# ucla-mobility/QuantV2X

Hardware: AMD Instinct MI355X
Metric: frames/sec/node (N-agent int8 BEV fusion) (higher is better)
Workload: dtype i8

## Files before the change

### include/qv2x.h

```cpp
#ifndef QV2X_H
#define QV2X_H

#include <stdint.h>

#ifdef __cplusplus
extern "C" {
#endif
#if defined(__GNUC__) || defined(__clang__)
#pragma GCC visibility push(default)
#endif

#define QV2X_OK 0
#define QV2X_EINVAL (-1)
#define QV2X_EALIGN (-2)
#define QV2X_MAX_GROUPS 4

const char* qv2x_last_error(void);
#define QV2X_ABI_VERSION 9
int qv2x_version(void);

int qv2x_fill_i8(int8_t* buf, int64_t bytes, int value, void* stream);

int64_t qv2x_voxelize_workspace_bytes(int n_points);
int qv2x_voxelize_f32(const float* points, int n_points, const float* lidar_range, const float* voxel_size, int agent,
                      int max_points, int max_voxels, void* workspace, int64_t workspace_bytes,
                      float* voxel_features, int32_t* voxel_coords, int32_t* voxel_num_points, int32_t* n_voxels, void* stream);

int64_t qv2x_voxelize_batch_workspace_bytes(int n_sweeps, const int32_t* n_points );
int qv2x_voxelize_batch_f32(const float* const* points , const int32_t* n_points , int n_sweeps,
                            const float* lidar_range, const float* voxel_size, int first_agent, int max_points, int capacity,
                            void* workspace, int64_t workspace_bytes, float* voxel_features, int32_t* voxel_coords,
                            int32_t* voxel_num_points, int32_t* voxel_counts, void* stream);

typedef struct {
    float w[64 * 10];
    float b[64];
    float d1, z1, d2, z2;
    float vox[3], off[3];
} qv2x_pfn_params;
int qv2x_pfn_scatter_i8(const float* voxel_features, const int32_t* voxel_coords, const int32_t* voxel_num_points,
                        int M, int max_points, const qv2x_pfn_params* params ,
                        int8_t* canvas, int N, int ny, int nx, void* stream);
int qv2x_pfn_unscatter_i8(const int32_t* voxel_coords, int M, int value, int8_t* canvas, int N, int ny, int nx, void* stream);

typedef struct {
    int32_t n, h, w, cin_total, stride, cout;
    int32_t ngroups;
    int32_t group_c0[QV2X_MAX_GROUPS], group_c[QV2X_MAX_GROUPS], group_zx[QV2X_MAX_GROUPS];
    int32_t out_ctotal, out_c0;
    int32_t relu;
    float out_delta, out_zp;
} qv2x_conv_desc;
int qv2x_conv3x3_i8(const qv2x_conv_desc* desc , const int8_t* in, const int8_t* w,
                    const float* scale, const int32_t* corr, const int32_t* aw, const float* bias,
                    int8_t* out, void* stream);

int qv2x_conv3x3_i8_wide_ok(const qv2x_conv_desc* desc );
int qv2x_conv3x3_i8_pack_wide(const qv2x_conv_desc* desc , const int8_t* w, int8_t* w_wide, void* stream);
int qv2x_conv3x3_i8_wide(const qv2x_conv_desc* desc , const int8_t* in, const int8_t* w_wide,
                         const float* scale, const int32_t* corr, const int32_t* aw, const float* bias,
                         int8_t* out, void* stream);

typedef struct {
    int32_t n, h, w;
    int32_t in_h, in_w;
    int32_t depth, stride0, relu;
    float out_delta[4], out_zp[4];
} qv2x_chain_desc;
int qv2x_conv3x3_i8_chain64(const qv2x_chain_desc* desc , const int8_t* in, const int8_t* w_chain,
                            const float* scale, const int32_t* corr, const int32_t* aw, const float* bias,
                            int8_t* out, void* stream);

typedef struct {
    int32_t n, h, w, cin, cout, s;
    int32_t in_zx;
    float in_delta;
    int32_t out_ctotal, out_c0, relu;
    float out_delta, out_zp;
    int32_t out_h, out_w;
} qv2x_deconv_desc;
int qv2x_deconv_i8(const qv2x_deconv_desc* desc , const int8_t* in, const float* w, const float* bias,
                   int8_t* out, void* stream);

int qv2x_deconv_i8_batch(const qv2x_deconv_desc* descs , int n, const int8_t* const* ins ,
                         const float* const* ws, const float* const* biases, int8_t* const* outs, void* stream);

typedef struct {
    int32_t n, h, w;
    int32_t levels, kc;
    int32_t in_zx;
    float in_delta;
    int32_t segs;
} qv2x_encode_desc;
int64_t qv2x_codebook_level_floats(int kc);
int qv2x_codebook_c2_f32(const float* codebook, int kc, float* c2, void* stream);
int qv2x_codebook_encode_f32(const qv2x_encode_desc* desc , const int8_t* in,
                             const float* const* level_weights ,
                             uint8_t* codes, void* stream);
int qv2x_codebook_encode_wave_f32(const qv2x_encode_desc* desc , const int8_t* in, const float* in_f32,
                                  const float* const* level_weights , uint8_t* codes, void* stream);

int qv2x_codebook_encode_collapsed_f32(const qv2x_encode_desc* desc , const int8_t* in, const float* g_packed, const float* bias,
                                       const float* tables, uint8_t* codes, void* stream);

int qv2x_codebook_encode_candidates_i8(const qv2x_encode_desc* desc , const int8_t* in, const int8_t* g_limbs, const double* bias_packed,
                                       const int32_t* tables, const float* tau , uint8_t* codes, uint32_t* list, uint32_t* counters,
                                       void* stream);
int qv2x_codebook_encode_listed_f32(const qv2x_encode_desc* desc , const int8_t* in, const float* const* level_weights ,
                                    const uint32_t* list, const uint32_t* list_count, uint8_t* codes, void* stream);

int qv2x_codebook_encode_candidates_seg_i8(const qv2x_encode_desc* desc , const int8_t* in, const int8_t* g_limbs, const double* bias_packed,
                                           const int32_t* tables, const float* tau , uint8_t* codes, uint32_t* list, uint32_t* counters,
                                           void* stream);

typedef struct {
    int32_t agents, h, w, levels, kc;
    int32_t max_cav, ego;
    int64_t code_agent_stride, code_level_stride;
    double h_metres, w_metres, discrete_ratio;
    int32_t fusion;
} qv2x_fuse_desc;
int qv2x_fuse_att_f32(const qv2x_fuse_desc* desc , const uint8_t* codes, const float* lut, const float* lut_bias,
                      const float* feats, const double* pairwise, float* fused, void* stream);

int qv2x_fuse_att_batch_f32(const qv2x_fuse_desc* desc , int n_scenes, const int64_t* scene_offset ,
                            const int32_t* scene_agents , const uint8_t* codes, const float* lut, const float* lut_bias,
                            const float* feats, const double* pairwise, float* fused, void* stream);

int qv2x_decode_lut_f32(const uint8_t* codes, int R, int levels, int kc, const float* lut, const float* lut_bias,
                        float* out, void* stream);

int qv2x_dequant_i8_f32(const int8_t* in, int n, int h, int w, int c, int zp, float delta, float* out, void* stream);

int qv2x_heads_f32(const float* x, int R, int hw, int cout, int cout_pad, const float* w, const float* bias,
                   const float* da, const float* za, float* out, void* stream);

int qv2x_fuse_heads_batch_f32(const qv2x_fuse_desc* desc , int n_scenes, const int64_t* scene_offset ,
                              const int32_t* scene_agents , const uint8_t* codes, const float* lut, const float* lut_bias,
                              const float* feats, const double* pairwise, int cout, int cout_pad, const float* w, const float* bias,
                              const float* da, const float* za, float* out, float* fused_tap, void* stream);

int qv2x_table_heads_f32(const uint8_t* codes, int R, int hw, int levels, int kc, int c0, int c1, const float* tables,
                         const float* bias, const float* da, const float* za, float* out0, float* out1, void* stream);

int qv2x_decode_heads_f32(const uint8_t* codes, int R, int hw, int levels, int kc, const float* lut, const float* lut_bias,
                          int cout, int cout_pad, const float* w, const float* bias, const float* da, const float* za,
                          float* out, void* stream);

int qv2x_single_heads_lut_f32(const uint8_t* codes, int R, int hw, int levels, int kc, int cout, const float* tables,
                              const float* bias, const float* da, const float* za, float* out, void* stream);

int qv2x_heads_pair_f32(const float* x, int R, int hw, int cout, int cout_pad, const float* w, const float* bias,
                        const float* da, const float* za, float* out,
                        const uint8_t* codes, int R1, int levels, int kc, const float* lut, const float* lut_bias,
                        int cout1, int cout_pad1, const float* w1, const float* bias1, const float* da1,
                        const float* za1, float* out1, void* stream);

typedef struct {
    int32_t h, w, anchors_per_cell, num_bins;
    float score_threshold, nms_threshold, dir_offset;
    float range[6];
    float transform[16];
    int32_t max_boxes;
    int32_t num_classes;
    int32_t range_xy_only;
    float max_extent, z_min, z_max;
} qv2x_postprocess_desc;
int64_t qv2x_postprocess_workspace_bytes(const qv2x_postprocess_desc* desc );
int qv2x_postprocess_f32(const qv2x_postprocess_desc* desc , const float* cls, const float* reg, const float* dir,
                         const float* anchors, void* workspace, int64_t workspace_bytes, float* out_corners,
                         float* out_scores, int32_t* out_labels, int32_t* out_count, void* stream);

int64_t qv2x_postprocess_batch_workspace_bytes(const qv2x_postprocess_desc* desc , int frames);
int qv2x_postprocess_batch_f32(const qv2x_postprocess_desc* desc , int frames, const float* cls, int64_t cls_frame_stride,
                               const float* reg, int64_t reg_frame_stride, const float* dir, int64_t dir_frame_stride,
                               const float* anchors, const float* transforms , void* workspace, int64_t workspace_bytes,
                               float* out_corners, float* out_scores, int32_t* out_labels, int32_t* out_count, void* stream);

int64_t qv2x_postprocess_late_workspace_bytes(const qv2x_postprocess_desc* desc , int ncav);
int qv2x_postprocess_late_f32(const qv2x_postprocess_desc* desc , int ncav, const float* const* cls, const float* const* reg,
                              const float* const* dir, const float* const* anchors, const float* transforms , void* workspace,
                              int64_t workspace_bytes, float* out_corners, float* out_scores, int32_t* out_labels, int32_t* out_count,
                              void* stream);

typedef struct {
    int32_t n, h, w;
    int32_t cin_total, cin0, cin;
    int32_t stride;
    int32_t cout;
    int32_t out_ctotal, out_c0, relu;
} qv2x_f32conv_desc;
int qv2x_conv3x3_f32(const qv2x_f32conv_desc* desc , const float* in, const float* w, const float* bias, float* out, void* stream);
int qv2x_deconv_f32(const qv2x_f32conv_desc* desc , const float* in, const float* w, const float* bias, float* out, void* stream);
int qv2x_pfn_scatter_f32(const float* voxel_features, const int32_t* voxel_coords, const int32_t* voxel_num_points, int M, int max_points,
                         const float* w, const float* b, const float* vox, const float* off, float* canvas, int N, int ny, int nx, void* stream);
int qv2x_codebook_encode_f32in(const qv2x_encode_desc* desc , const float* in, const float* const* level_weights ,
                               uint8_t* codes, void* stream);

int qv2x_pyramid_weighted_fuse_f32(const qv2x_fuse_desc* desc , int channels, const float* feats, const float* score,
                                   const double* pairwise, float* out, void* stream);


typedef struct {
    int32_t n, h, w, cin, cout, stride;
    int32_t mode, relu;
    int32_t out_ctotal, out_c0;
    float out_delta, out_zp;
    int32_t res_zx;
    float res_delta;
} qv2x_conv1x1_desc;
int qv2x_conv1x1_i8(const qv2x_conv1x1_desc* desc , const int8_t* in, const int8_t* w_frag, const float* scale,
                    const int32_t* corr, const int32_t* aw, const float* bias, const void* res, void* out, void* stream);

typedef struct {
    int32_t n, h, w, c, cg, stride, relu;
    float out_delta, out_zp;
} qv2x_gconv_desc;
int qv2x_gconv3x3_i8(const qv2x_gconv_desc* desc , const int8_t* in, const int8_t* w_frag, const float* scale,
                     const int32_t* corr, const int32_t* aw, const float* bias, int8_t* out, void* stream);

typedef struct {
    int32_t n, h, w, planes, width, cg;
    int32_t in_zx;
    float in_delta;
    float delta1, zp1, delta2, zp2, out_delta, out_zp;
} qv2x_bottleneck_desc;
int qv2x_bottleneck_i8(const qv2x_bottleneck_desc* desc , const int8_t* x, const int8_t* const* w, const float* const* scale,
                       const int32_t* const* corr, const int32_t* const* aw, const float* const* bias, int8_t* out, void* stream);

int qv2x_conv3x3_i8_res(const qv2x_conv_desc* desc , const int8_t* in, const int8_t* w, const float* scale, const int32_t* corr,
                        const int32_t* aw, const float* bias, int res_mode, const void* res, int res_zx, float res_delta,
                        int8_t* out, void* stream);

int qv2x_deconv_f32in(const qv2x_deconv_desc* desc , const float* in, const float* w, const float* bias, int8_t* out, void* stream);

int qv2x_codebook_decode_f32(const uint8_t* codes, int64_t agent_stride, int64_t level_stride, int agents, int hw, int levels,
                             int kc, int d, const float* lut, const float* bias, float* out, void* stream);

int64_t qv2x_codebook64_level_floats(int kc);
int qv2x_codebook64_c2_f32(const float* codebook, int kc, float* c2, void* stream);
int qv2x_codebook_encode64_f32(const qv2x_encode_desc* desc , int cin_total, const int8_t* in,
                               const float* const* level_weights , uint8_t* codes, void* stream);

int qv2x_codebook_encode64_f32in(const qv2x_encode_desc* desc , int cin_total, const float* in,
                                 const float* const* level_weights , uint8_t* codes, void* stream);

int qv2x_add_relu_f32(const float* a, const float* b, float* out, int64_t count, void* stream);
int qv2x_occ_sigmoid_f32(const float* in, int n, int h, int w, int c_total, float* occ, float* score, void* stream);
int qv2x_pyramid_weighted_fuse_f32p(const qv2x_fuse_desc* desc , int channels, const float* feats, const float* score,
                                    const double* pairwise, float* out, void* stream);

typedef struct {
    int32_t n, h, w, c;
    int32_t aw, corr;
    float scale, bias, out_delta, out_zp;
} qv2x_occ_desc;
int qv2x_occ_score_i8(const qv2x_occ_desc* desc , const int8_t* in, const int8_t* w, const float* score_lut, float* score,
                      uint8_t* occ_code, void* stream);

int qv2x_pyramid_weighted_fuse_i8(const qv2x_fuse_desc* desc , int channels, const int8_t* feats, int in_zx, float in_delta,
                                  const float* score, const double* pairwise, float* out, void* stream);

typedef struct {
    int32_t subm;
    int32_t k[3], s[3], p[3];
    int32_t in_shape[3], out_shape[3];
    int32_t agents, cin, cout;
    int32_t cap_in, cap_out;
    float out_delta, out_zp;
} qv2x_spconv_desc;
int qv2x_mean_vfe_f32(const float* voxel_features, const int32_t* voxel_num_points, const int32_t* n_voxels , int cap,
                      int max_points, float* out, void* stream);
int qv2x_sp_index_scatter(const int32_t* coords, const int32_t* n_rows , int cap, int agents, int D, int H, int W,
                          int32_t* volume, int set, void* stream);
int64_t qv2x_sp_out_sites_workspace_bytes(const qv2x_spconv_desc* desc );
int qv2x_sp_out_sites(const qv2x_spconv_desc* desc , const int32_t* in_coords, const int32_t* n_in, int32_t* out_volume,
                      int32_t* out_coords, int32_t* n_out, void* workspace, int64_t workspace_bytes, void* stream);
int qv2x_sp_rulebook(const qv2x_spconv_desc* desc , const int32_t* out_coords, const int32_t* n_out, const int32_t* in_volume,
                     int32_t* nbr, void* stream);
int qv2x_sp_conv_f32in(const qv2x_spconv_desc* desc , const float* feat, const int32_t* nbr, const int32_t* n_out, const float* w,
                       const float* bn_g, const float* bn_h, int8_t* out, void* stream);
int qv2x_sp_conv_i8(const qv2x_spconv_desc* desc , const int8_t* in, const int32_t* nbr, const int32_t* n_out, const int8_t* w_frag,
                    const float* scale, const int32_t* corr, const int32_t* aw, const float* bn_g, const float* bn_h, int8_t* out, void* stream);
int qv2x_sp_to_bev_i8(const int8_t* feat, const int32_t* coords, const int32_t* n_rows , int cap, int c, int c_padded, int agents,
                      int D, int H, int W, int fill, int8_t* bev, void* stream);

#define QV2X_COMM_ID_BYTES 128
int qv2x_comm_unique_id(void* id );
int qv2x_comm_init(const void* id , int world, int rank, void** comm);
int qv2x_comm_destroy(void* comm);
int qv2x_allgather_codes(void* comm, const uint8_t* send, uint8_t* recv, int64_t bytes_per_rank, void* stream);

int qv2x_pairwise_from_poses_f64(const uint8_t* gathered, int world, int64_t agent_stride_bytes, int64_t pose_offset_bytes,
                                 int max_cav, double* pairwise, void* stream);
int qv2x_pairwise_from_poses_batch_f64(const uint8_t* gathered, int world, int64_t agent_stride_bytes, int64_t pose_offset_bytes,
                                       int frames, int64_t frame_stride_bytes, int max_cav, double* pairwise, void* stream);

#define QV2X_WIRE_F32 0
#define QV2X_WIRE_U8 1
int qv2x_fuse_att_band_f32(const qv2x_fuse_desc* desc , int n_scenes, const int64_t* scene_offset ,
                           const int32_t* scene_agents , const uint8_t* codes, const float* lut, const float* lut_bias,
                           const float* feats, const double* pairwise, int64_t cell0, int64_t n_cells, float* fused, void* stream);
int qv2x_heads_band(const float* x, int n_scenes, int64_t n_cells, int cout, int cout_pad, const float* w, const float* bias,
                    const float* da, const float* za, int wire, const float* da_host , void* out, void* stream);
int qv2x_fuse_heads_band(const qv2x_fuse_desc* desc , int n_scenes, const int64_t* scene_offset ,
                         const int32_t* scene_agents , const uint8_t* codes, const float* lut, const float* lut_bias,
                         const float* feats, const double* pairwise, int64_t cell0, int64_t n_cells, int cout, int cout_pad,
                         const float* w, const float* bias, const float* da, const float* za, int wire, const float* da_host ,
                         void* out, float* fused_tap, void* stream);
int qv2x_assemble_bands(const uint8_t* slabs, int world, int64_t slab_bytes, int frames, int cout, int h, int w, int wire,
                        const float* da, const float* za, float* out, void* stream);

typedef struct {
    int32_t frames;
    int32_t det_cap;
    int32_t gt_cap;
    int32_t n_classes;
    int32_t n_ranges;
    int32_t n_thresholds;
    float ranges[4][2];
    float thresholds[4];
} qv2x_eval_desc;
int64_t qv2x_eval_workspace_bytes(const qv2x_eval_desc* desc );
int qv2x_eval_tp_fp_f32(const qv2x_eval_desc* desc , const float* det_corners, const float* det_scores, const int32_t* det_labels,
                        const int32_t* det_count, const float* gt_corners, const int32_t* gt_labels, const int32_t* gt_count,
                        void* workspace, int64_t workspace_bytes, int32_t* out_order, float* out_scores, uint8_t* out_flags,
                        int32_t* out_match, int32_t* out_gt, void* stream);

typedef struct {
    int32_t frames;
    int32_t agents;
    int32_t obj_cap;
    int32_t gt_cap;
    int32_t row_floats;
    int32_t order;
    int32_t mode;
    int32_t range_xy_only;
    float range[6];
    float iou_threshold;
} qv2x_gt_desc;
int qv2x_gt_boxes_f32(const qv2x_gt_desc* desc , const float* boxes, const uint8_t* mask, const int32_t* ids, const float* transforms,
                      const int32_t* agent_counts, float* gt_corners, int32_t* gt_labels, int32_t* gt_ids, int32_t* gt_counts,
                      int32_t* gt_totals, void* stream);

#if defined(__GNUC__) || defined(__clang__)
#pragma GCC visibility pop
#endif
#ifdef __cplusplus
}
#endif
#endif
```

### quantv2x_amd/csrc/codebook_encode_cand.hip

```cpp
#include "common.h"

namespace qv2x {
namespace {

struct CandArgs {
    const int8_t* in; const int8_t* gpack; const double* bias; const int* tables;
    uint8_t* codes; unsigned* list; unsigned* counters;
    float tau[3][3];
    int n, h, w, hw, M, levels, kc, ke, zx, gbytes, tbytes;
    float delta;
};

constexpr int NPF = 8;
constexpr int LIMBS = 3;
template <int V> struct IC { static constexpr int value = V; };

__device__ __forceinline__ double shfl_xor_f64(double v, int m) {
    const long long b = __builtin_bit_cast(long long, v);
    const int lo = __shfl_xor((int)b, m), hi = __shfl_xor((int)(b >> 32), m);
    return __builtin_bit_cast(double, ((long long)hi << 32) | (unsigned)lo);
}

template <int CT, int SEGS, int PACK>
__global__ __launch_bounds__(256) __attribute__((amdgpu_waves_per_eu(1, 1))) void encode_candidates_kernel(const CandArgs a) {
    const int lane = threadIdx.x & 63, wave = __builtin_amdgcn_readfirstlane(threadIdx.x >> 6), j = lane & 31, hf = lane >> 5;
    const int m0 = ((int)blockIdx.x * 4 + wave) * (32 * CT);

    v4i xb[CT][8];
    int m[CT];
    float n0[CT], n1[CT];
#pragma unroll
    for (int ct = 0; ct < CT; ++ct) {
        m[ct] = m0 + 32 * ct + j;
        const int mc = m[ct] < a.M ? m[ct] : a.M - 1;
        const int img = mc / a.hw, rem = mc - img * a.hw, y = rem / a.w, x = rem - y * a.w;
        const int8_t* px = a.in + ((size_t)(img * (a.h + 2) + y + 1) * (a.w + 2) + x + 1) * 256 + 16 * hf;
#pragma unroll
        for (int s = 0; s < 8; ++s) xb[ct][s] = *(const v4i*)(px + 32 * s);
        unsigned s1 = 0, s2 = 0, sad = 0;
        const unsigned zx4 = (unsigned)a.zx * 0x01010101u;
#pragma unroll
        for (int s = 0; s < 8; ++s)
#pragma unroll
            for (int d = 0; d < 4; ++d) {
                const unsigned u = (unsigned)xb[ct][s][d] ^ 0x80808080u;
                s1 = __builtin_amdgcn_udot4(u, 0x01010101u, s1, false);
                s2 = __builtin_amdgcn_udot4(u, u, s2, false);
                sad = __builtin_amdgcn_sad_u8(u, zx4, sad);
            }
        s1 += __shfl_xor(s1, 32); s2 += __shfl_xor(s2, 32); sad += __shfl_xor(sad, 32);
        const int n2 = (int)s2 - 2 * a.zx * (int)s1 + 256 * a.zx * a.zx;
        n0[ct] = a.delta * sqrtf((float)n2);
        n1[ct] = (float)sad;
    }

    const __amdgpu_buffer_rsrc_t grs = __builtin_amdgcn_make_buffer_rsrc((void*)a.gpack, 0, a.gbytes, 0x00020000);
    int wo = 0;
    const int loff = lane * 16;
    auto gload = [&](int f) __attribute__((always_inline)) { return (v4i)__builtin_amdgcn_raw_buffer_load_b128(grs, loff, wo + f * 1024, 0); };
    v4i ring[NPF];
#pragma unroll
    for (int i = 0; i < NPF; ++i) ring[i] = gload(i);

    const __amdgpu_buffer_rsrc_t brs = __builtin_amdgcn_make_buffer_rsrc((void*)a.bias, 0, a.levels * a.ke * 8, 0x00020000);
    const __amdgpu_buffer_rsrc_t trs = __builtin_amdgcn_make_buffer_rsrc((void*)a.tables, 0, a.tbytes, 0x00020000);
    int o[2][SEGS][CT] = {};
    int first[CT];
#pragma unroll
    for (int ct = 0; ct < CT; ++ct) first[ct] = 3;
    const int ntile = a.kc >> 5;
    const int tsz = a.ke * a.ke;
    auto level = [&](auto lc) __attribute__((always_inline)) {
        constexpr int l = decltype(lc)::value;
        bool weak_l[CT];
#pragma unroll
        for (int ct = 0; ct < CT; ++ct) weak_l[ct] = false;
        auto segment = [&](auto sc) __attribute__((always_inline)) {
        constexpr int sg = decltype(sc)::value;
        double best[CT], second[CT];
#pragma unroll
        for (int ct = 0; ct < CT; ++ct) best[ct] = second[ct] = 1.0e300;
        v4i qb[2][2], qt[2][l > 0 ? l * SEGS : 1][CT];
        auto issue = [&](int T, int g, int slot) __attribute__((always_inline)) {
            const int col = sg * a.kc + 32 * T + 8 * g;
            const int kofs = l * a.ke + col;
            qb[slot][0] = (v4i)__builtin_amdgcn_raw_buffer_load_b128(brs, 32 * hf, kofs * 8, 0);
            qb[slot][1] = (v4i)__builtin_amdgcn_raw_buffer_load_b128(brs, 32 * hf + 16, kofs * 8, 0);
#pragma unroll
            for (int ct = 0; ct < CT; ++ct) {
#pragma unroll
                for (int jj = 0; jj < l; ++jj)
#pragma unroll
                    for (int sp = 0; sp < SEGS; ++sp)
                        qt[slot][jj * SEGS + sp][ct] = (v4i)__builtin_amdgcn_raw_buffer_load_b128(trs, o[jj][sp][ct], ((l * (l - 1) / 2 + jj) * tsz + col) * 4, 0);
            }
        };
#pragma unroll 1
        for (int T = 0; T < ntile; ++T) {
            v16i acc[LIMBS][CT];
#pragma unroll
            for (int lb = 0; lb < LIMBS; ++lb)
#pragma unroll
                for (int ct = 0; ct < CT; ++ct)
#pragma unroll
                    for (int r = 0; r < 16; ++r) acc[lb][ct][r] = 0;
#pragma unroll
            for (int f = 0; f < LIMBS * 8; ++f) {
                const v4i A = ring[f % NPF];
#pragma unroll
                for (int ct = 0; ct < CT; ++ct) acc[f >> 3][ct] = __builtin_amdgcn_mfma_i32_32x32x32_i8(A, xb[ct][f & 7], acc[f >> 3][ct], 0, 0, 0);
                ring[f % NPF] = gload(f + NPF);
                if (f == LIMBS * 8 - 6) issue(T, 0, 0);
                __builtin_amdgcn_sched_barrier(0);
            }
            wo += LIMBS * 8 * 1024;
#pragma unroll
            for (int g = 0; g < 4; ++g) {
                if (g < 3) issue(T, g + 1, (g + 1) & 1);
                __builtin_amdgcn_sched_barrier(0);
                const int sl = g & 1;
                double b[4];
                b[0] = __builtin_bit_cast(double, ((unsigned long long)(unsigned)qb[sl][0][1] << 32) | (unsigned)qb[sl][0][0]);
                b[1] = __builtin_bit_cast(double, ((unsigned long long)(unsigned)qb[sl][0][3] << 32) | (unsigned)qb[sl][0][2]);
                b[2] = __builtin_bit_cast(double, ((unsigned long long)(unsigned)qb[sl][1][1] << 32) | (unsigned)qb[sl][1][0]);
                b[3] = __builtin_bit_cast(double, ((unsigned long long)(unsigned)qb[sl][1][3] << 32) | (unsigned)qb[sl][1][2]);
#pragma unroll
                for (int ct = 0; ct < CT; ++ct) {
#pragma unroll
                    for (int e = 0; e < 4; ++e) {
                        const int r = 4 * g + e;
                        int lo = (acc[1][ct][r] << 8) + acc[0][ct][r];
#pragma unroll
                        for (int q = 0; q < l * SEGS; ++q) lo += qt[sl][q][ct][e];
                        double c = __builtin_fma((double)lo, (double)PACK, b[e]);
                        c = __builtin_fma((double)acc[2][ct][r], 65536.0 * PACK, c);
                        second[ct] = fmin(second[ct], fmax(best[ct], c));
                        best[ct] = fmin(best[ct], c);
                    }
                }
                __builtin_amdgcn_sched_barrier(0);
            }
        }
#pragma unroll
        for (int ct = 0; ct < CT; ++ct) {
            const double ob = shfl_xor_f64(best[ct], 32), os = shfl_xor_f64(second[ct], 32);
            const double nb = fmin(best[ct], ob), ns = fmin(fmax(best[ct], ob), fmin(second[ct], os));
            const int c = (int)((long long)nb & (PACK - 1));
            if (l < 2) o[l < 2 ? l : 0][sg][ct] = ((sg * a.kc + c) * a.ke + 4 * hf) * 4;
            const float t = ((a.tau[l][0] + a.tau[l][1] * n0[ct]) + (a.tau[l][2] * n0[ct]) * n0[ct]) + n1[ct];
            weak_l[ct] |= !(ns - nb > (double)PACK * (double)ceilf(t) + (double)(PACK - 1));
            if (hf == 0 && m[ct] < a.M) a.codes[(size_t)(l * SEGS + sg) * a.M + m[ct]] = (uint8_t)c;
        }
        };
        segment(IC<0>{});
        if constexpr (SEGS > 1) segment(IC<1>{});
#pragma unroll
        for (int ct = 0; ct < CT; ++ct)
            if (weak_l[ct] && first[ct] == 3) first[ct] = l;
    };
    level(IC<0>{});
    if (a.levels > 1) level(IC<1>{});
    if (a.levels > 2) level(IC<2>{});
    unsigned long long mask[3][CT];
    unsigned cnt[3] = {0, 0, 0};
#pragma unroll
    for (int c = 0; c < 3; ++c)
#pragma unroll
        for (int ct = 0; ct < CT; ++ct) {
            mask[c][ct] = __builtin_amdgcn_ballot_w64(first[ct] == c && hf == 0 && m[ct] < a.M);
            cnt[c] += (unsigned)__builtin_popcountll(mask[c][ct]);
        }
    __shared__ unsigned wcnt[4][3], wbase[3];
    if (lane == 0) { wcnt[wave][0] = cnt[0]; wcnt[wave][1] = cnt[1]; wcnt[wave][2] = cnt[2]; }
    __syncthreads();
    if (threadIdx.x < 3) {
        const unsigned tot = wcnt[0][threadIdx.x] + wcnt[1][threadIdx.x] + wcnt[2][threadIdx.x] + wcnt[3][threadIdx.x];
        wbase[threadIdx.x] = tot ? atomicAdd(a.counters + 1 + threadIdx.x, tot) : 0u;
        if (tot) atomicAdd(a.counters, tot);
    }
    __syncthreads();
    unsigned base[3];
#pragma unroll
    for (int c = 0; c < 3; ++c) {
        base[c] = wbase[c];
        for (int w2 = 0; w2 < wave; ++w2) base[c] += wcnt[w2][c];
    }
#pragma unroll
    for (int c = 0; c < 3; ++c) {
        unsigned at = __builtin_amdgcn_readfirstlane(base[c]);
#pragma unroll
        for (int ct = 0; ct < CT; ++ct) {
            if (first[ct] == c && hf == 0 && m[ct] < a.M)
                a.list[(size_t)c * a.M + at + (unsigned)__builtin_popcountll(mask[c][ct] & ((1ull << lane) - 1ull))] = (unsigned)m[ct];
            at += (unsigned)__builtin_popcountll(mask[c][ct]);
        }
    }
}

__global__ void zero_counters_kernel(unsigned* c) { if (threadIdx.x < 4) c[threadIdx.x] = 0; }

template <int CT, int SEGS, int PACK>
void launch(const CandArgs& a, hipStream_t st) {
    encode_candidates_kernel<CT, SEGS, PACK><<<(a.M + 128 * CT - 1) / (128 * CT), 256, 0, st>>>(a);
}

template <int PACK, int MAX_SEGS>
int candidates(const char* me, const qv2x_encode_desc* d, const int8_t* in, const int8_t* g_limbs, const double* bias_packed, const int32_t* tables,
               const float* tau, uint8_t* codes, uint32_t* list, uint32_t* counters, void* stream) {
    if (!d || !in || !g_limbs || !bias_packed || !tau || !codes || !list || !counters) return fail(QV2X_EINVAL, "%s: null pointer", me);
    if (d->n <= 0 || d->h <= 0 || d->w <= 0 || d->levels < 1 || d->levels > 3) return fail(QV2X_EINVAL, "%s: 1..3 levels", me);
    const int segs = d->segs ? d->segs : 1;
    if (segs < 1 || segs > MAX_SEGS) return fail(QV2X_EINVAL, "%s: seg_num 1 .. %d (got %d; the exact entry takes seg_num 1 | 2 | 4)", me, MAX_SEGS, d->segs);
    if (d->kc < 32 || d->kc > PACK || d->kc % 32 || (segs > 1 && d->kc % 64))
        return fail(QV2X_EINVAL, "%s: dict_size a multiple of 32 up to %d (of 64 with two segments; got %d x %d)", me, PACK, segs, d->kc);
    if (d->levels > 1 && !tables) return fail(QV2X_EINVAL, "%s: the residual levels need their tables", me);
    if (d->in_zx < 0 || d->in_zx > 255) return fail(QV2X_EINVAL, "%s: in_zx outside 0..255", me);
    if (((uintptr_t)in & 15) || ((uintptr_t)g_limbs & 15) || ((uintptr_t)tables & 15) || ((uintptr_t)bias_packed & 7))
        return fail(QV2X_EALIGN, "%s: 16-byte aligned maps, limbs and tables", me);
    CandArgs a;
    a.in = in; a.gpack = g_limbs; a.bias = bias_packed; a.tables = tables; a.codes = codes; a.list = list; a.counters = counters;
    for (int l = 0; l < 3; ++l)
        for (int i = 0; i < 3; ++i) a.tau[l][i] = l < d->levels ? tau[l * 3 + i] : 0.0f;
    a.n = d->n; a.h = d->h; a.w = d->w; a.hw = d->h * d->w; a.M = d->n * a.hw; a.levels = d->levels; a.kc = d->kc; a.ke = segs * d->kc; a.zx = d->in_zx;
    a.gbytes = d->levels * (a.ke / 32) * LIMBS * 8 * 1024;
    a.tbytes = (d->levels > 1 ? d->levels * (d->levels - 1) / 2 : 1) * a.ke * a.ke * 4;
    a.delta = d->in_delta;
    hipStream_t st = (hipStream_t)stream;
    zero_counters_kernel<<<1, 64, 0, st>>>(counters);
    int dev = 0, cus = 256, v = 0;
    if (hipGetDevice(&dev) == hipSuccess && hipDeviceGetAttribute(&v, hipDeviceAttributeMultiprocessorCount, dev) == hipSuccess && v > 0) cus = v;
    const bool large = a.M >= 4 * cus * 32 * (segs == 2 ? 3 : 4) * 2;
    if (segs == 1) large ? launch<4, 1, PACK>(a, st) : launch<2, 1, PACK>(a, st);
    else if constexpr (MAX_SEGS > 1) large ? launch<3, 2, PACK>(a, st) : launch<2, 2, PACK>(a, st);
    return hip_check(hipGetLastError(), me);
}

}
}

extern "C" int qv2x_codebook_encode_candidates_i8(const qv2x_encode_desc* d, const int8_t* in, const int8_t* g_limbs, const double* bias_packed,
                                                  const int32_t* tables, const float* tau, uint8_t* codes, uint32_t* list, uint32_t* counters,
                                                  void* stream) {
    return qv2x::candidates<128, 1>("qv2x_codebook_encode_candidates_i8", d, in, g_limbs, bias_packed, tables, tau, codes, list, counters, stream);
}

extern "C" int qv2x_codebook_encode_candidates_seg_i8(const qv2x_encode_desc* d, const int8_t* in, const int8_t* g_limbs, const double* bias_packed,
                                                      const int32_t* tables, const float* tau, uint8_t* codes, uint32_t* list, uint32_t* counters,
                                                      void* stream) {
    return qv2x::candidates<256, 2>("qv2x_codebook_encode_candidates_seg_i8", d, in, g_limbs, bias_packed, tables, tau, codes, list, counters, stream);
}
```

### quantv2x_amd/csrc/pfn_scatter.hip

```cpp
#include "common.h"

namespace qv2x {

constexpr int PFN_PB = 4, PFN_PQ = 2;

__global__ __launch_bounds__(256, 6) void pfn_scatter_kernel(const float4* __restrict__ vf, const int4* __restrict__ coords,
                                                          const int* __restrict__ npts, int M, int P,
                                                          const qv2x_pfn_params prm, int8_t* __restrict__ canvas,
                                                          int N, int ny, int nx) {
    const int lane = threadIdx.x & 63;
    int m0 = (blockIdx.x * 4 + (threadIdx.x >> 6)) * PFN_PB;
    m0 = __builtin_amdgcn_readfirstlane(m0);
    if (m0 >= M) return;

    int4 c[PFN_PB];
    int np[PFN_PB];
    float4 q[PFN_PB][PFN_PQ];
#pragma unroll
    for (int j = 0; j < PFN_PB; ++j) {
        const int m = m0 + j < M ? m0 + j : M - 1;
        c[j] = coords[m];
        np[j] = npts[m];
    }
#pragma unroll
    for (int j = 0; j < PFN_PB; ++j) {
        const int m = m0 + j < M ? m0 + j : M - 1;
#pragma unroll
        for (int p = 0; p < PFN_PQ; ++p) q[j][p] = vf[(size_t)m * P + (p < P ? p : P - 1)];
    }
    float w[10];
#pragma unroll
    for (int k = 0; k < 10; ++k) w[k] = prm.w[lane * 10 + k];
    const float b = prm.b[lane];

#pragma unroll
    for (int j = 0; j < PFN_PB; ++j) {
        if (m0 + j >= M) break;
        const float4* pts = vf + (size_t)(m0 + j) * P;
        const int real = np[j] < P ? np[j] : P;
        float sx = 0.f, sy = 0.f, sz = 0.f;
#pragma unroll
        for (int p = 0; p < PFN_PQ; ++p)
            if (p < real) { sx += q[j][p].x; sy += q[j][p].y; sz += q[j][p].z; }
        for (int p = PFN_PQ; p < real; ++p) {
            const float4 t = pts[p];
            sx += t.x; sy += t.y; sz += t.z;
        }
        const float n = (float)np[j];
        const float mx = sx / n, my = sy / n, mz = sz / n;
        const float cx = (float)c[j].w * prm.vox[0] + prm.off[0];
        const float cy = (float)c[j].z * prm.vox[1] + prm.off[1];
        const float cz = (float)c[j].y * prm.vox[2] + prm.off[2];

        float ymax = -INFINITY;
        auto point = [&](const float4 t) __attribute__((always_inline)) {
            const float f[10] = {t.x, t.y, t.z, t.w, t.x - mx, t.y - my, t.z - mz, t.x - cx, t.y - cy, t.z - cz};
            float acc = 0.0f;
#pragma unroll
            for (int k = 0; k < 10; ++k) acc = fmaf(f[k], w[k], acc);
            ymax = fmaxf(ymax, acc + b);
        };
#pragma unroll
        for (int p = 0; p < PFN_PQ; ++p)
            if (p < real) point(q[j][p]);
        for (int p = PFN_PQ; p < real; ++p) point(pts[p]);
        if (real < P) ymax = fmaxf(ymax, b);

        const float q1 = q_code(ymax, prm.d1, prm.z1);
        float y1 = (q1 - prm.z1) * prm.d1;
        y1 = fmaxf(y1, 0.0f);
        const int code = (int)q_code(y1, prm.d2, prm.z2);

        if (c[j].x < 0 || c[j].x >= N || c[j].z < 0 || c[j].z >= ny || (c[j].y + c[j].w) < 0 || (c[j].y + c[j].w) >= nx) continue;
        const size_t cell = ((size_t)c[j].x * (ny + 2) + (c[j].z + 1)) * (nx + 2) + (size_t)(c[j].y + c[j].w + 1);
        canvas[cell * 64 + lane] = (int8_t)(code - 128);
    }
}

constexpr int PFN_R = 8;
#ifndef PFN_NQ
#define PFN_NQ 2
#endif

__global__ __launch_bounds__(256, 4) void pfn_scatter16_kernel(const float4* __restrict__ vf, const int4* __restrict__ coords,
                                                            const int* __restrict__ npts, int M, int P,
                                                            const qv2x_pfn_params prm, int8_t* __restrict__ canvas,
                                                            int N, int ny, int nx, int rounds) {
    __shared__ float wl[640 + 64];
    __shared__ uint8_t lut[256];
    for (int i = threadIdx.x; i < 640; i += 256) wl[i] = prm.w[i];
    if (threadIdx.x < 64) wl[640 + threadIdx.x] = prm.b[threadIdx.x];
    {
        const float q1 = (float)(threadIdx.x ^ 0x80);
        float y1 = (q1 - prm.z1) * prm.d1;
        y1 = fmaxf(y1, 0.0f);
        lut[threadIdx.x] = (uint8_t)((int)q_code(y1, prm.d2, prm.z2) - 128);
    }
    const float rd1 = 1.0f / prm.d1;
    __syncthreads();
    const int sub = threadIdx.x & 15, slot = threadIdx.x >> 4;
    float w[4][10], b[4];
#pragma unroll
    for (int c = 0; c < 4; ++c) {
#pragma unroll
        for (int k = 0; k < 10; ++k) w[c][k] = wl[(sub * 4 + c) * 10 + k];
        b[c] = wl[640 + sub * 4 + c];
    }
    const int mbase = blockIdx.x * (16 * rounds) + slot;

    auto header = [&](int m, int4& c, int& np, float4 (&q)[PFN_NQ]) __attribute__((always_inline)) {
        const int mm = m < M ? m : M - 1;
        c = coords[mm];
        np = npts[mm];
#pragma unroll
        for (int p = 0; p < PFN_NQ; ++p) q[p] = vf[(size_t)mm * P + (p < P ? p : P - 1)];
    };
    int4 c, cn;
    int np, npn;
    float4 q[PFN_NQ], qn[PFN_NQ];
    header(mbase, c, np, q);
#pragma unroll 1
    for (int r = 0; r < rounds; ++r) {
        const int m = mbase + r * 16;
        if (r + 1 < rounds) header(m + 16, cn, npn, qn);
        if (m < M) {
            const float4* pts = vf + (size_t)m * P;
            const int real = np < P ? np : P;
            float sx = 0.f, sy = 0.f, sz = 0.f;
#pragma unroll
            for (int p = 0; p < PFN_NQ; ++p)
                if (p < real) { sx += q[p].x; sy += q[p].y; sz += q[p].z; }
            for (int p = PFN_NQ; p < real; ++p) {
                const float4 t = pts[p];
                sx += t.x; sy += t.y; sz += t.z;
            }
            const float n = (float)np;
            const float mx = sx / n, my = sy / n, mz = sz / n;
            const float cx = (float)c.w * prm.vox[0] + prm.off[0];
            const float cy = (float)c.z * prm.vox[1] + prm.off[1];
            const float cz = (float)c.y * prm.vox[2] + prm.off[2];
            float ymax[4] = {-INFINITY, -INFINITY, -INFINITY, -INFINITY};
            auto point = [&](const float4 t) __attribute__((always_inline)) {
                const float f[10] = {t.x, t.y, t.z, t.w, t.x - mx, t.y - my, t.z - mz, t.x - cx, t.y - cy, t.z - cz};
#pragma unroll
                for (int ch = 0; ch < 4; ++ch) {
                    float acc = 0.0f;
#pragma unroll
                    for (int k = 0; k < 10; ++k) acc = fmaf(f[k], w[ch][k], acc);
                    ymax[ch] = fmaxf(ymax[ch], acc + b[ch]);
                }
            };
#pragma unroll
            for (int p = 0; p < PFN_NQ; ++p)
                if (p < real) point(q[p]);
            for (int p = PFN_NQ; p < real; ++p) point(pts[p]);
            if (real < P) {
#pragma unroll
                for (int ch = 0; ch < 4; ++ch) ymax[ch] = fmaxf(ymax[ch], b[ch]);
            }
            const unsigned c1 = (unsigned)q_pack4_div(ymax[0], ymax[1], ymax[2], ymax[3], prm.d1, rd1, prm.z1);
            const unsigned word = (unsigned)lut[c1 & 0xff] | ((unsigned)lut[(c1 >> 8) & 0xff] << 8) | ((unsigned)lut[(c1 >> 16) & 0xff] << 16) |
                                  ((unsigned)lut[c1 >> 24] << 24);
            if (!(c.x < 0 || c.x >= N || c.z < 0 || c.z >= ny || (c.y + c.w) < 0 || (c.y + c.w) >= nx)) {
                const size_t cell = ((size_t)c.x * (ny + 2) + (c.z + 1)) * (nx + 2) + (size_t)(c.y + c.w + 1);
                *(unsigned*)(canvas + cell * 64 + sub * 4) = word;
            }
        }
        c = cn; np = npn;
#pragma unroll
        for (int p = 0; p < PFN_NQ; ++p) q[p] = qn[p];
    }
}

__global__ __launch_bounds__(256) void pfn_unscatter_kernel(const int4* __restrict__ coords, int M, int value4, int8_t* __restrict__ canvas,
                                                            int N, int ny, int nx) {
    const long long id = (long long)blockIdx.x * 256 + threadIdx.x;
    const int m = (int)(id >> 2), piece = (int)(id & 3);
    if (m >= M) return;
    const int4 c = coords[m];
    if (c.x < 0 || c.x >= N || c.z < 0 || c.z >= ny || (c.y + c.w) < 0 || (c.y + c.w) >= nx) return;
    const size_t cell = ((size_t)c.x * (ny + 2) + (c.z + 1)) * (nx + 2) + (size_t)(c.y + c.w + 1);
    v4i v; v[0] = v[1] = v[2] = v[3] = value4;
    *(v4i*)(canvas + cell * 64 + piece * 16) = v;
}

}

extern "C" int qv2x_pfn_unscatter_i8(const int32_t* voxel_coords, int M, int value, int8_t* canvas, int N, int ny, int nx, void* stream) {
    using namespace qv2x;
    if (M == 0) return QV2X_OK;
    if (!voxel_coords || !canvas) return fail(QV2X_EINVAL, "qv2x_pfn_unscatter_i8: null pointer");
    if (M < 0 || N <= 0 || ny <= 0 || nx <= 0 || value < -128 || value > 127) return fail(QV2X_EINVAL, "qv2x_pfn_unscatter_i8: bad sizes / value");
    if (((uintptr_t)voxel_coords & 15) || ((uintptr_t)canvas & 15)) return fail(QV2X_EALIGN, "qv2x_pfn_unscatter_i8: coords / canvas must be 16-byte aligned");
    const int b = value & 0xff, v4 = b | (b << 8) | (b << 16) | (b << 24);
    const long long threads = (long long)M * 4;
    pfn_unscatter_kernel<<<(unsigned)((threads + 255) / 256), 256, 0, (hipStream_t)stream>>>((const int4*)voxel_coords, M, v4, canvas, N, ny, nx);
    return hip_check(hipGetLastError(), "qv2x_pfn_unscatter_i8 launch");
}

extern "C" int qv2x_pfn_scatter_i8(const float* voxel_features, const int32_t* voxel_coords, const int32_t* voxel_num_points,
                                   int M, int max_points, const qv2x_pfn_params* params, int8_t* canvas, int N, int ny, int nx,
                                   void* stream) {
    using namespace qv2x;
    if (M == 0) return QV2X_OK;
    if (!voxel_features || !voxel_coords || !voxel_num_points || !params || !canvas)
        return fail(QV2X_EINVAL, "qv2x_pfn_scatter_i8: null pointer");
    if (M < 0 || max_points <= 0 || N <= 0 || ny <= 0 || nx <= 0) return fail(QV2X_EINVAL, "qv2x_pfn_scatter_i8: bad sizes");
    if (((uintptr_t)voxel_features & 15) || ((uintptr_t)voxel_coords & 15)) return fail(QV2X_EALIGN, "qv2x_pfn_scatter_i8: inputs must be 16-byte aligned");
    int form = 16;
#ifdef QV2X_DEV_KNOBS
    static const int form_env = getenv("QV2X_PFN_FORM") ? atoi(getenv("QV2X_PFN_FORM")) : 16;
    form = form_env;
#endif
    if (form == 64)
        pfn_scatter_kernel<<<(M + 4 * PFN_PB - 1) / (4 * PFN_PB), 256, 0, (hipStream_t)stream>>>((const float4*)voxel_features, (const int4*)voxel_coords,
                                                                         voxel_num_points, M, max_points, *params, canvas, N, ny, nx);
    else {
        static const int cus = [] {
            int dev = 0, v = 0;
            return hipGetDevice(&dev) == hipSuccess && hipDeviceGetAttribute(&v, hipDeviceAttributeMultiprocessorCount, dev) == hipSuccess && v > 0 ? v : 256;
        }();
        int rounds = M / (16 * 8 * cus);
        rounds = rounds < 1 ? 1 : (rounds > PFN_R ? PFN_R : rounds);
        pfn_scatter16_kernel<<<(M + 16 * rounds - 1) / (16 * rounds), 256, 0, (hipStream_t)stream>>>((const float4*)voxel_features, (const int4*)voxel_coords,
                                                                          voxel_num_points, M, max_points, *params, canvas, N, ny, nx, rounds);
    }
    return hip_check(hipGetLastError(), "qv2x_pfn_scatter_i8 launch");
}
```

### quantv2x_amd/encode_two_stage.py

```python
from typing import Dict

import numpy as np

U = 2.0 ** -24
LIMBS = 3
G_MAX_INT = 2 ** 23 - 2 ** 15 - 2 ** 7 - 1


def _sn(m):
    return float(np.linalg.norm(m, 2)) if m.size else 0.0


def _kappa(w, block=8):
    k = w.shape[1]
    return float(sum(min(block, k - i0) * _sn(w[:, :min(k, i0 + block)]) for i0 in range(0, k, block)))


class _Aff:

    def __init__(self, p=0.0, r=0.0):
        self.p, self.r = float(p), float(r)

    def __add__(self, o):
        return _Aff(self.p + o.p, self.r + o.r)

    def scale(self, c):
        return _Aff(self.p * c, self.r * c)


def encode_error_bound(state: Dict[str, np.ndarray], levels: int, delta: float, segs: int = 1):
    g = lambda l, n: state[f"codebook/{l}/{n}"].astype(np.float64)
    u1 = U / (1.0 - U)
    ub = u1 / (1.0 - 256.0 * u1)
    eye = np.eye(256)
    A, shift, back = eye.copy(), np.zeros(256), []
    srcs = [(eye.copy(), _Aff(U, 0.0), "x0 = fl(n * delta)")]
    ea, eb, ec, report = [], [], [], []

    def offset(shift, back):
        return float(np.linalg.norm(shift) + sum(sum(float(n.max()) for n in np.split(np.linalg.norm(g(j, "codebook") @ B.T, axis=1), segs))
                                                 for j, B in enumerate(back)))

    def norm_bound(A, shift, back, srcs):
        d = _Aff()
        for M, e, _ in srcs:
            d = d + e.scale(_sn(M))
        return _Aff(_sn(A), offset(shift, back)) + d

    def layer(W, b, vin: _Aff):
        return _Aff(ub * _kappa(W) * vin.p, ub * (256.0 * float(np.linalg.norm(b)) + _kappa(W) * vin.r) + 1e-30)

    for l in range(levels):
        S, bs, Q, bq, Cb = g(l, "stage_w"), g(l, "stage_b"), g(l, "qhead_w"), g(l, "qhead_b"), g(l, "codebook")
        vx = norm_bound(A, shift, back, srcs)
        srcs = [(S @ M, e, n) for M, e, n in srcs] + [(eye.copy(), layer(S, bs, vx), f"stage{l}")]
        A, shift, back = S @ A, S @ shift + bs, [S @ B for B in back]
        vz = norm_bound(A, shift, back, srcs)
        sq = [(Q @ M, e, n) for M, e, n in srcs] + [(eye.copy(), layer(Q, bq, vz), f"qhead{l}")]
        vq = norm_bound(Q @ A, Q @ shift + bq, [Q @ B for B in back], sq)
        cn = np.linalg.norm(Cb, axis=1)
        cmax, c2max = float(cn.max()), float((cn ** 2).max())
        e = _Aff()
        for M, eps, name in sq:
            wpair = 0.0
            for K in np.split(Cb @ M, segs):
                gram = K @ K.T
                dg = np.diag(gram)
                wpair = max(wpair, float(np.sqrt(max(0.0, (dg[:, None] + dg[None, :] - 2.0 * gram).max()))))
            e = e + eps.scale(2.0 * wpair)
            report.append((l, name, wpair, eps.p, eps.r))
        e = e + vq.scale(2.0 * 2.0 * 256.0 * ub * cmax)
        e = e + vq.scale(2.0 * 2.0 * U * cmax * (1.0 + 256.0 * ub))
        fin = 2.0 * U * (2.0 + U)
        x2 = fin * (1.0 + 2.0 ** -17)
        ea.append(e.r + (fin * (1.0 + 1e-5) + 2.0 * 67.0 * U) * c2max + x2 * vq.r * vq.r)
        eb.append(e.p + x2 * 2.0 * vq.p * vq.r)
        ec.append(x2 * vq.p * vq.p)
        if l < levels - 1:
            Lh, bl = g(l, "lhead_w"), g(l, "lhead_b")
            srcs = [(Lh @ M, e_, n) for M, e_, n in srcs] + [(eye.copy(), layer(Lh, bl, vz), f"lhead{l}")]
            A, shift, back = Lh @ A, Lh @ shift + bl, [Lh @ B for B in back] + [eye.copy()]
            vn = norm_bound(A, shift, back, srcs)
            srcs = srcs + [(eye.copy(), vn.scale(U / (1.0 - U)), f"sub{l}")]
    host = 1.0 + 1e-6
    return np.array(ea) * host, np.array(eb) * host, np.array(ec) * host, report


def pack_factor(segs: int, kc: int) -> int:
    return 128 if segs == 1 and kc <= 128 else 256


CANDIDATE_ENTRY = {128: "qv2x_codebook_encode_candidates_i8", 256: "qv2x_codebook_encode_candidates_seg_i8"}


def candidate_tables(state: Dict[str, np.ndarray], levels: int, in_delta: float, in_zx: int, segs: int = 1) -> Dict[str, np.ndarray]:
    from .engine import collapse_encoder_f64
    G, gb, tabs = collapse_encoder_f64(state, levels)
    ke = G.shape[0] // levels
    kc = ke // segs
    if any(state[f"codebook/{l}/codebook"].shape[0] != ke for l in range(levels)):
        raise ValueError("two-stage encode: every level needs the same dict_size")
    if segs == 1:
        if kc % 32 or kc > 256 or levels > 3:
            raise ValueError("two-stage encode: dict_size 32 | 64 | 96 | 128 | ... | 256, up to three levels")
    elif segs != 2 or kc * segs != ke or kc % 64 or kc > 256 or levels > 3:
        raise ValueError("two-stage encode: seg_num 1 | 2, dict_size a multiple of 64 up to 256 with two segments, up to three levels")
    n_t = segs * max(levels - 1, 0)
    tlim = 2.0 ** 29 / max(2, n_t)
    blim = 2.0 ** 44 if pack_factor(segs, kc) == 128 else 2.0 ** 43
    gs = float(in_delta) * G
    tmax = max([float(np.abs(t).max()) for t in tabs.values()] + [0.0])
    h = max(float(np.abs(gs).max()) / G_MAX_INT, tmax / (tlim - 2.0), float(np.abs(gb).max()) / (blim - 2.0 ** 32))
    gi = np.rint(gs / h).astype(np.int64)
    limbs, rest = [], gi.copy()
    for _ in range(LIMBS):
        d = ((rest + 128) % 256) - 128
        limbs.append(d.astype(np.int8))
        rest = (rest - d) // 256
    if rest.any():
        raise ValueError("two-stage encode: G on the grid does not fit the candidate stage's int8 limbs")
    bias = np.rint(gb / h).astype(np.int64) + (128 - int(in_zx)) * gi.sum(1)
    tables = np.stack([np.rint(tabs[(l, j)] / h) for l in range(levels) for j in range(l)]) if levels > 1 else np.zeros((1, ke, ke))
    if np.abs(tables).max() >= tlim or np.abs(bias).max() >= blim:
        raise ValueError("two-stage encode: table / bias entries leave the fixed-point range of the candidate stage")
    lane = np.arange(64)
    score = (np.arange(levels * ke // 32)[:, None, None, None] * 32 + (lane & 31)[None, None, :, None])
    chan = (32 * np.arange(8)[None, :, None, None] + 16 * (lane >> 5)[None, None, :, None] + np.arange(16)[None, None, None, :])
    packed = np.stack([lb[score, chan] for lb in limbs], axis=1)
    packed = packed.reshape(levels, ke // 32, LIMBS, 8, 64, 16)
    ea, eb, ec, report = encode_error_bound(state, levels, in_delta, segs)
    fp = 1.0 + 1e-4
    tau = np.zeros((levels, 3))
    for l in range(levels):
        own = 1.0 + segs * l + 2.0
        tau[l] = [(ea[l] / h + own) * fp, eb[l] / h * fp, ec[l] / h * fp]
    return {"gpack": np.ascontiguousarray(packed, dtype=np.int8), "bias": np.ascontiguousarray(bias, dtype=np.int64),
            "tables": np.ascontiguousarray(tables, dtype=np.int32), "tau": np.ascontiguousarray(tau, dtype=np.float32), "h": h,
            "g_int": gi, "bound": (ea, eb, ec), "report": report, "segs": segs, "kc": kc, "pack": pack_factor(segs, kc)}


def candidate_emulate(codes_u8: np.ndarray, tabs: Dict[str, np.ndarray], in_delta: float, in_zx: int):
    gi, bias, tables, tau, h = tabs["g_int"], tabs["bias"], tabs["tables"], tabs["tau"], tabs["h"]
    levels = tau.shape[0]
    segs = int(tabs.get("segs", 1))
    ke = gi.shape[0] // levels
    kc = ke // segs
    P = float(tabs.get("pack", 128))
    b = codes_u8.astype(np.float64) - 128.0
    s = b @ gi.astype(np.float64).T + bias.astype(np.float64)[None]
    n = codes_u8.astype(np.int64) - int(in_zx)
    n1, n2 = np.abs(n).sum(1), (n * n).sum(1)
    n0 = (np.float32(in_delta) * np.sqrt(n2.astype(np.float32))).astype(np.float32)
    out = np.zeros((levels * segs, codes_u8.shape[0]), np.uint8)
    flags = np.zeros((levels * segs, codes_u8.shape[0]), bool)
    gaps = np.zeros((levels * segs, codes_u8.shape[0]))
    for l in range(levels):
        sc = s[:, l * ke:(l + 1) * ke].copy()
        for j in range(l):
            for sp in range(segs):
                sc += tables[l * (l - 1) // 2 + j][sp * kc + out[j * segs + sp].astype(np.int64)].astype(np.float64)
        t = (((tau[l, 0] + tau[l, 1] * n0) + (tau[l, 2] * n0) * n0) + n1.astype(np.float32)).astype(np.float32)
        assert t.dtype == np.float32 and n0.dtype == np.float32
        t = t.astype(np.float64)
        for sg in range(segs):
            v = sc[:, sg * kc:(sg + 1) * kc]
            order = np.argsort(v, axis=1, kind="stable")
            best, second = np.take_along_axis(v, order[:, :1], 1)[:, 0], np.take_along_axis(v, order[:, 1:2], 1)[:, 0]
            p = l * segs + sg
            out[p] = order[:, 0]
            k2 = order[:, 1]
            flags[p] = (P * second + k2) - (P * best + out[p]) <= P * np.ceil(t) + (P - 1.0)
            gaps[p] = (second - best) * h
    return out, flags.any(0), flags, gaps
```

### quantv2x_amd/engine.py

```python
from __future__ import annotations

import ctypes as C
from typing import Dict, List, Optional

import numpy as np
import torch
import torch.nn as nn

from . import lib as L
from .ptq_state import export_ptq_state, load_ptq_state

_HEADS = ("cls_head", "reg_head", "dir_head")


def _dev(a: np.ndarray, dev) -> torch.Tensor:
    return torch.from_numpy(np.ascontiguousarray(a)).to(dev).contiguous()


def _pack_k4(w: np.ndarray) -> np.ndarray:
    j, k = w.shape
    assert k % 4 == 0
    return np.ascontiguousarray(w.T.reshape(k // 4, 4, j).transpose(0, 2, 1), dtype=np.float32)


def decode_tables(state: Dict[str, np.ndarray], levels: int, width: int = 256):
    g = lambda l, n: state[f"codebook/{l}/{n}"].astype(np.float64)
    tables, const, chain = [], np.zeros(width), np.eye(width)
    for l in range(levels):
        front = chain @ g(l, "restore_w")
        tables.append((front @ g(l, "dqhead_w") @ g(l, "codebook").T).T)
        const = const + front @ g(l, "dqhead_b") + chain @ g(l, "restore_b")
        if l < levels - 1:
            const = const + front @ g(l, "side_b")
            chain = front @ g(l, "side_w")
    return np.ascontiguousarray(np.stack(tables), dtype=np.float32), np.ascontiguousarray(const, dtype=np.float32)


def collapse_encoder_f64(state: Dict[str, np.ndarray], levels: int):
    g = lambda l, n: state[f"codebook/{l}/{n}"].astype(np.float64)
    kc = int(state["codebook/0/codebook"].shape[0])
    front, shift = np.eye(256), np.zeros(256)
    back = []
    G, gb, tables = [], [], {}
    for l in range(levels):
        Ws, bs, Wq, bq, Cb = g(l, "stage_w"), g(l, "stage_b"), g(l, "qhead_w"), g(l, "qhead_b"), g(l, "codebook")
        Gp = -2.0 * Cb @ Wq @ Ws
        gp = (Cb * Cb).sum(1) - 2.0 * Cb @ (Wq @ bs + bq)
        G.append(Gp @ front)
        gb.append(Gp @ shift + gp)
        for j, Bj in enumerate(back):
            tables[(l, j)] = -(Gp @ Bj @ g(j, "codebook").T).T
        if l < levels - 1:
            A = g(l, "lhead_w") @ Ws
            d = g(l, "lhead_w") @ bs + g(l, "lhead_b")
            front, shift = A @ front, A @ shift + d
            back = [A @ Bj for Bj in back] + [np.eye(256)]
    return np.concatenate(G), np.concatenate(gb), tables


def collapse_encoder(state: Dict[str, np.ndarray], levels: int, in_delta: float, in_zx: int):
    Gall, gall, tables = collapse_encoder_f64(state, levels)
    kc = Gall.shape[0] // levels
    bias = gall + in_delta * (0.0 - in_zx) * Gall.sum(1)
    Gs = in_delta * Gall
    nct = levels * kc // 32
    lane = np.arange(64)
    col = (np.arange(nct)[:, None, None] * 32 + (lane & 31)[None, None, :])
    k = (2 * np.arange(128)[None, :, None] + (lane >> 5)[None, None, :])
    packed = Gs[col, k]
    tab = np.stack([tables[(l, j)] for l in range(levels) for j in range(l)]) if levels > 1 else np.zeros((1, kc, kc))
    return (np.ascontiguousarray(packed, dtype=np.float32), np.ascontiguousarray(bias, dtype=np.float32), np.ascontiguousarray(tab, dtype=np.float32))


def _pack_k4p(w: np.ndarray) -> np.ndarray:
    return np.ascontiguousarray(_pack_k4(w)[:, :, [0, 2, 1, 3]])


def _pack_wave(w: np.ndarray) -> np.ndarray:
    j, k = w.shape
    assert k == 256
    if j % 64:
        w = np.concatenate([w, np.zeros((64 - j % 64, k), w.dtype)])
    return np.ascontiguousarray(w.reshape(-1, 2, 32, 32, 4, 2).transpose(0, 3, 1, 5, 2, 4), dtype=np.float32)


ENC_WAVE_PAD = 16 * 256


def _pack_wave_seg(cb: np.ndarray, segs: int) -> np.ndarray:
    ke, k = cb.shape
    kc, d = ke // segs, 256 // segs
    assert k == 256 and segs in (2, 4) and kc % 32 == 0
    blocks = np.stack([cb[sg * kc:(sg + 1) * kc, sg * d:(sg + 1) * d] for sg in range(segs)])
    b = blocks.reshape(segs // 2, 2, kc // 32, 32, d // 8, 4, 2)
    return np.ascontiguousarray(b.transpose(0, 2, 4, 1, 6, 3, 5), dtype=np.float32)


def wave_section(stage_w, qhead_w, lhead_w, cb, segs: int = 1) -> np.ndarray:
    cbs = _pack_wave(cb) if segs == 1 else _pack_wave_seg(cb, segs)
    sec = np.concatenate([_pack_wave(stage_w).reshape(-1), _pack_wave(qhead_w).reshape(-1), cbs.reshape(-1), _pack_wave(lhead_w).reshape(-1)])
    full = 3 * 65536 + (cb.shape[0] + 63) // 64 * 64 * 256
    return np.concatenate([sec, np.zeros(full - sec.size + ENC_WAVE_PAD, np.float32)])


class _ConvLayer:

    def __init__(self, state, name, in_groups, stride, dev, pad_cin=0, pad_cout=0):
        code = state[name + "/w_code"]
        dw = state[name + "/w_delta"].astype(np.float32)
        zw = state[name + "/w_zp"].astype(np.int64)
        bias_np = state[name + "/bias"].astype(np.float32)
        if pad_cin > code.shape[1]:
            fill = np.broadcast_to(np.clip(zw, 0, 255).astype(np.uint8)[:, None, None, None], (code.shape[0], pad_cin - code.shape[1], 3, 3))
            code = np.concatenate([code, fill], axis=1)
        if pad_cout > code.shape[0]:
            extra = pad_cout - code.shape[0]
            code = np.concatenate([code, np.full((extra,) + code.shape[1:], 128, np.uint8)])
            dw, zw = np.concatenate([dw, np.ones(extra, np.float32)]), np.concatenate([zw, np.full(extra, 128, np.int64)])
            bias_np = np.concatenate([bias_np, np.zeros(extra, np.float32)])
        cout = code.shape[0]
        ws = code.astype(np.int64) - 128
        aw = 128 - zw
        parts, corr, scale = [], [], []
        for (c0, c, dx, zx) in in_groups:
            blk = ws[:, c0:c0 + c].transpose(0, 2, 3, 1).reshape(cout, -1)
            parts.append(blk)
            ax = 128 - int(zx)
            corr.append(ax * blk.sum(axis=1) + blk.shape[1] * ax * aw)
            scale.append(np.float32(dx) * dw)
        self.name, self.stride, self.cout = name, stride, cout
        self.groups = [(int(c0), int(c), int(zx)) for (c0, c, _, zx) in in_groups]
        self.w = _dev(np.concatenate(parts, axis=1).astype(np.int8), dev)
        self.w_wide = None
        self.scale = _dev(np.stack(scale).astype(np.float32), dev)
        self.corr = _dev(np.stack(corr).astype(np.int32), dev)
        self.aw = _dev(aw.astype(np.int32), dev)
        self.bias = _dev(bias_np, dev)
        self.out_q = (float(np.float32(state[name + "/a_delta"])), int(state[name + "/a_zp"]))
        assert np.abs(np.stack(corr)).max() < 2 ** 31


class _ChainLayers:
    MAX_DEPTH = 4

    @staticmethod
    def eligible(convs) -> bool:
        return (1 <= len(convs) <= _ChainLayers.MAX_DEPTH and all(c.cout == 64 and len(c.groups) == 1 and c.groups[0][1] == 64 for c in convs)
                and all(c.stride == 1 for c in convs[1:]))

    def __init__(self, convs, dev):
        self.convs = convs
        self.name = convs[-1].name
        packed = []
        for c in convs:
            w = c.w.cpu().numpy().reshape(2, 32, 9, 2, 2, 16)
            packed.append(w.transpose(0, 2, 3, 4, 1, 5))
        self.w = _dev(np.stack(packed).astype(np.int8), dev)
        cat = lambda ts: torch.cat([t.reshape(-1) for t in ts]).contiguous()
        self.scale, self.corr = cat([c.scale for c in convs]), cat([c.corr for c in convs])
        self.aw, self.bias = cat([c.aw for c in convs]), cat([c.bias for c in convs])
        self.stride0 = convs[0].stride
        self.out_q = convs[-1].out_q


class _DeconvLayer:
    def __init__(self, state, name, in_q, dev):
        code = state[name + "/w_code"].astype(np.float32)
        dw = state[name + "/w_delta"].astype(np.float32).reshape(-1, 1, 1, 1)
        zw = state[name + "/w_zp"].astype(np.float32).reshape(-1, 1, 1, 1)
        wdeq = ((code - zw) * dw).astype(np.float32)
        cin, cout, s, _ = wdeq.shape
        cols = wdeq.transpose(0, 2, 3, 1).reshape(cin, s * s * cout)
        self.w = _dev(_pack_k4p(cols.T), dev)
        self.bias = _dev(state[name + "/bias"].astype(np.float32), dev)
        self.name, self.cin, self.cout, self.s, self.in_q = name, cin, cout, s, in_q
        self.out_q = (float(np.float32(state[name + "/a_delta"])), int(state[name + "/a_zp"]))


class _Heads:

    def __init__(self, state, suffix, dev):
        ws, bs, das, zas = [], [], [], []
        for h in _HEADS:
            n = h + suffix
            code = state[n + "/w_code"].astype(np.float32).reshape(state[n + "/w_code"].shape[0], -1)
            w = ((code - state[n + "/w_zp"].astype(np.float32)[:, None]) * state[n + "/w_delta"].astype(np.float32)[:, None])
            ws.append(w.astype(np.float32))
            bs.append(state[n + "/bias"].astype(np.float32))
            off = bool(state[n + "/a_off"])
            das.append(np.full(w.shape[0], -1.0 if off else float(np.float32(state[n + "/a_delta"])), np.float32))
            zas.append(np.full(w.shape[0], 0.0 if off else float(state[n + "/a_zp"]), np.float32))
        self.splits = [w.shape[0] for w in ws]
        self.cout = sum(self.splits)
        self.cout_pad = (self.cout + 31) // 32 * 32
        if self.cout_pad > 96:
            raise NotImplementedError("heads: at most 96 stacked output channels")
        pad = self.cout_pad - self.cout
        w = np.concatenate(ws + [np.zeros((pad, 256), np.float32)])
        self.w = _dev(_pack_k4p(w), dev)
        self.bias = _dev(np.concatenate(bs + [np.zeros(pad, np.float32)]), dev)
        self.da = _dev(np.concatenate(das + [np.full(pad, -1.0, np.float32)]), dev)
        self.za = _dev(np.concatenate(zas + [np.zeros(pad, np.float32)]), dev)
        self._w_np, self._b_np = np.concatenate(ws).astype(np.float64), np.concatenate(bs).astype(np.float64)
        self.da_np = np.ascontiguousarray(np.concatenate(das))
        self.lut_tables = None

    def collapse_over_decode(self, lut: np.ndarray, lut_bias: np.ndarray, dev):
        t = np.einsum("lkd,cd->lkc", lut.astype(np.float64), self._w_np)
        b = lut_bias.astype(np.float64) @ self._w_np.T + self._b_np
        self.lut_tables = (_dev(t.astype(np.float32), dev), _dev(b.astype(np.float32), dev))


def scene_layout(data_dict: dict, n_total: int):
    pairwise = data_dict["pairwise_t_matrix"]
    if pairwise.dtype != torch.float64 or not pairwise.is_contiguous():
        pairwise = pairwise.to(torch.float64).contiguous()
    if pairwise.shape[0] == 1:
        return pairwise, [n_total]
    rl = data_dict["record_len"]
    if isinstance(rl, torch.Tensor) and rl.is_cuda and torch.cuda.is_current_stream_capturing():
        raise ValueError("record_len on the GPU cannot be read during HIP-graph capture: pass a CPU tensor")
    return pairwise, [int(v) for v in (rl.tolist() if isinstance(rl, torch.Tensor) else rl)]


def split_heads(preds: torch.Tensor, splits, suffix: str = "") -> dict:
    c, r, _ = splits
    out = {"cls_preds" + suffix: preds[:, :c], "reg_preds" + suffix: preds[:, c:c + r], "dir_preds" + suffix: preds[:, c + r:]}
    if not suffix:
        out["preds_tensor"] = preds
    return out


def capture_call(call):
    side = torch.cuda.Stream()
    side.wait_stream(torch.cuda.current_stream())
    with torch.cuda.stream(side):
        for _ in range(2):
            call()
    torch.cuda.current_stream().wait_stream(side)
    graph = torch.cuda.CUDAGraph()
    with torch.cuda.graph(graph):
        out = call()

    def replay():
        graph.replay()
        return out
    replay.graph = graph
    return replay


def capture_forward(module: nn.Module, data_dict: dict):
    rl = data_dict.get("record_len")
    if data_dict["pairwise_t_matrix"].shape[0] > 1 and isinstance(rl, torch.Tensor) and rl.is_cuda:
        data_dict = dict(data_dict, record_len=rl.cpu())
    return capture_call(lambda: module.forward(data_dict))


def assemble_heter_codes(owner: str, engines: dict, slot_cache: dict, agents: list, data_dict: dict, encode, taps: Optional[dict]) -> torch.Tensor:
    unknown = sorted(set(agents) - set(engines))
    if unknown:
        raise NotImplementedError(f"{owner}: no engine for modality {unknown}")
    slots = slot_cache.get(tuple(agents))
    if slots is None:
        if torch.cuda.is_current_stream_capturing():
            raise L.Qv2xError(f"{owner}: agent layout {agents} is new and the stream is capturing -- its slot indices are an H2D copy; "
                              "run one eager forward of this layout first (capture does)")
        slots = {m: torch.as_tensor([i for i, a in enumerate(agents) if a == m], dtype=torch.int64, device=e.dev) for m, e in engines.items()}
        slot_cache[tuple(agents)] = slots
    e = next(iter(engines.values()))
    n_total, hw, lv = len(agents), e.fh * e.fw, e.levels
    enc = torch.empty((lv, n_total * hw), dtype=torch.uint8, device=e.dev)
    for m, eng in engines.items():
        k = int(slots[m].numel())
        if not k:
            continue
        mt = {} if taps is not None else None
        codes = encode(eng, data_dict["inputs_" + m], k, mt).view(lv, k, hw)
        enc.view(lv, n_total, hw).index_copy_(1, slots[m], codes)
        if taps is not None:
            taps["modality/" + m] = mt
    return enc


class DeployedModel(nn.Module):
    fuse_heads_min_tiles = 4 * 1280
    fuse_heads_max_agents = 4
    single_agent_tables = True
    band_one_launch = None
    _band_rows = None
    table_heads = None

    def __init__(self, state: Dict[str, np.ndarray], device="cuda", emit_single_preds: Optional[bool] = None):
        super().__init__()
        lut, lut_bias = self._setup_common(state, device, emit_single_preds)
        s, dev = state, self.dev

        self.encoder_kind = str(s["meta/encoder"]) if "meta/encoder" in s else "point_pillar"
        if self.encoder_kind == "second":
            last = int(s["second/n_layers"]) - 1
            q = (float(np.float32(s[f"second/{last}/a_delta"])), int(s[f"second/{last}/a_zp"]))
            self.canvas_c, self.canvas_q, self.pfn = int(s["meta/canvas_channels"]), q, None
            self.second: Dict[int, object] = {}
            self.second_max_voxels, self.second_max_points = 70000, 5
        else:
            n = "encoder_m1.pillar_vfe.pfn_layers.0.linear"
            wq = ((s[n + "/w_code"].astype(np.float32) - s[n + "/w_zp"].astype(np.float32)[:, None])
                  * s[n + "/w_delta"].astype(np.float32)[:, None]).astype(np.float32)
            if wq.shape != (64, 10):
                raise NotImplementedError("deployed PFN expects Linear(10 -> 64)")
            p = L.PfnParams()
            p.w[:] = wq.reshape(-1).tolist()
            p.b[:] = s[n + "/bias"].astype(np.float32).tolist()
            p.d1, p.z1 = float(np.float32(s[n + "/a_delta"])), float(s[n + "/a_zp"])
            p.d2, p.z2 = float(np.float32(s["pfn/a2_delta"])), float(s["pfn/a2_zp"])
            p.vox[:] = [float(np.float32(v)) for v in s["meta/voxel"]]
            p.off[:] = [float(np.float32(v)) for v in s["meta/offset"]]
            self.pfn = p
            q = (p.d2, int(p.z2))
            self.canvas_c, self.canvas_q = 64, q

        self.blocks: List[List[_ConvLayer]] = []
        self.chains: List[Optional[_ChainLayers]] = []
        self.deblocks: List[_DeconvLayer] = []
        cat_groups, c0 = [], 0
        cin = self.canvas_c
        for lvl in range(len(self.layer_nums)):
            convs = []
            for i in range(self.layer_nums[lvl] + 1):
                layer = _ConvLayer(s, f"backbone_m1.blocks.{lvl}.{i + 1}", [(0, cin, q[0], q[1])],
                                   self.strides[lvl] if i == 0 else 1, dev)
                convs.append(layer)
                q, cin = layer.out_q, layer.cout
            self.blocks.append(convs)
            self.chains.append(_ChainLayers(convs, dev) if _ChainLayers.eligible(convs) else None)
            de = _DeconvLayer(s, f"backbone_m1.deblocks.{lvl}.0", q, dev)
            self.deblocks.append(de)
            cat_groups.append((c0, de.cout, de.out_q[0], de.out_q[1]))
            c0 += de.cout
        self.cat_channels = c0
        self.shrink0 = _ConvLayer(s, "shrinker_m1.layers.0.double_conv.0", cat_groups, 1, dev)
        self.shrink1 = _ConvLayer(s, "shrinker_m1.layers.0.double_conv.1",
                                  [(0, self.shrink0.cout, *self.shrink0.out_q)], 1, dev)
        if self.shrink1.cout != 256:
            raise NotImplementedError("deployed path expects a 256-channel shared feature")
        self.compress = bool(s.get("meta/compress", False))
        self.final = self.shrink1
        if self.compress:
            if self.has_codebook:
                raise NotImplementedError("deployed path: compressor and codebook together")
            narrow = int(s["compressor.encoder.0/w_code"].shape[0])
            pad = (narrow + 63) // 64 * 64
            self.comp = [_ConvLayer(s, "compressor.encoder.0", [(0, 256, *self.shrink1.out_q)], 1, dev, pad_cout=pad)]
            self.comp.append(_ConvLayer(s, "compressor.decoder.0", [(0, pad, *self.comp[0].out_q)], 1, dev, pad_cin=pad))
            self.comp.append(_ConvLayer(s, "compressor.decoder.1", [(0, 256, *self.comp[1].out_q)], 1, dev))
            self.comp_channels = narrow
            self.final = self.comp[-1]
        self.heads = _Heads(s, "", dev)
        self.heads_single = _Heads(s, "_single", dev) if (self.emit_single and "cls_head_single/w_code" in s) else None
        self.single_by_tables = (self.heads_single is not None and self.has_codebook and self.levels <= 4
                                 and self.levels * self.kc * self.heads_single.cout * 4 <= 60 * 1024)
        self.single_by_global_tables = (not self.single_by_tables and self.heads_single is not None and self.has_codebook and self.levels <= 16
                                        and self.heads_single.cout % 4 == 0 and self.heads_single.cout <= 128)
        if self.single_by_tables or self.single_by_global_tables:
            self.heads_single.collapse_over_decode(lut, lut_bias, dev)
        self.table_heads = None
        if self.has_codebook:
            sets = [self.heads] + ([self.heads_single] if self.heads_single is not None else [])
            ct = sum(h.cout for h in sets)
            ct4 = (ct + 3) // 4 * 4
            st = ct4 if (ct4 // 4) % 2 else ct4 + 4
            in_lds = self.levels <= 4 and (self.levels * self.kc * st + 4 * ct4) * 4 <= 160 * 1024
            if in_lds or (self.levels <= 16 and ct % 4 == 0 and ct <= 128):
                t = np.concatenate([np.einsum("lkd,cd->lkc", lut.astype(np.float64), h._w_np) for h in sets], axis=2)
                b = np.concatenate([lut_bias.astype(np.float64) @ h._w_np.T + h._b_np for h in sets])
                cat = lambda name: torch.cat([getattr(h, name)[:h.cout] for h in sets]).contiguous()
                self.table_heads = (_dev(t.astype(np.float32), dev), _dev(b.astype(np.float32), dev), cat("da"), cat("za"),
                                    self.heads.cout, self.heads_single.cout if self.heads_single is not None else 0)
        self._bufs: Dict[int, dict] = {}
        self.use_wide_conv, self.batch_deconvs, self.use_chains = True, True, True
        self.chain_max_agents = 1

    def _setup_common(self, state: Dict[str, np.ndarray], device, emit_single_preds: Optional[bool]):
        self.lib = L.load()
        if not torch.cuda.is_available():
            raise L.Qv2xError(f"{type(self).__name__} needs an MI355X (torch.cuda.is_available() is False)")
        self.state, self.dev = state, torch.device(device)
        s, dev = state, self.dev
        if str(s.get("meta/fusion_method", "att")) not in ("att", "max"):
            raise NotImplementedError(f"deployed path: fusion_method {s['meta/fusion_method']!r} ('att' = AttFusion and 'max' = MaxFusion are built here)")
        self.fusion = 1 if str(s.get("meta/fusion_method", "att")) == "max" else 0
        self.nx, self.ny, _ = (int(v) for v in s["meta/grid"])
        self.hm, self.wm = (float(v) for v in s["meta/HW_metres"])
        self.ratio = float(s["meta/discrete_ratio"])
        self.layer_nums = [int(v) for v in s["meta/layer_nums"]]
        self.strides = [int(v) for v in s["meta/layer_strides"]]
        self.ups = [int(v) for v in s["meta/upsample_strides"]]
        self.has_codebook = bool(s["meta/has_codebook"])
        self.emit_single = bool(s["meta/supervise_single"]) if emit_single_preds is None else bool(emit_single_preds)
        lut = lut_bias = None
        if self.has_codebook:
            self.enc_levels, self.segs = int(s["meta/codebook_levels"]), int(s.get("meta/codebook_segs", 1))
            self.levels = self.enc_levels * self.segs
            self.ke = int(s["codebook/0/codebook"].shape[0])
            self.kc = self.ke // self.segs
            if self.ke > 512 or self.kc > 256:
                raise NotImplementedError(f"deployed codebook path: seg_num * dict_size <= 512, dict_size <= 256 (got {self.segs} x {self.kc}): "
                                          "the encode kernels' tile budget (qv2x_codebook_encode_f32)")
            lut, lut_bias = decode_tables(s, self.enc_levels)
            lut = lut.reshape(self.levels, self.kc, lut.shape[-1])
            self.lut = _dev(lut, dev)
            self.lut_bias = _dev(lut_bias, dev)
            self.level_blobs = [self._level_blob(l) for l in range(self.enc_levels)]
            self.level_ptrs = (C.c_void_p * self.enc_levels)(*[b.data_ptr() for b in self.level_blobs])
        self._collapsed, self._two_stage, self.two_stage_refused = None, None, None
        self.encode_form = "auto"
        self.encode_mode = "two_stage" if self.two_stage_supported() else "exact"
        return lut, lut_bias

    def _level_blob(self, l: int) -> torch.Tensor:
        s, kc = self.state, self.ke
        g = lambda n: s[f"codebook/{l}/{n}"].astype(np.float32)
        zeros_w, zeros_b = np.zeros((64, 256, 4), np.float32), np.zeros(256, np.float32)
        last = f"codebook/{l}/lhead_w" not in s
        cb = g("codebook")
        parts = [_pack_k4p(g("stage_w")), g("stage_b"), _pack_k4p(g("qhead_w")), g("qhead_b"),
                 zeros_w if last else _pack_k4p(g("lhead_w")), zeros_b if last else g("lhead_b"),
                 _pack_k4p(cb), cb, np.zeros(kc, np.float32)]
        flat = np.concatenate([p.reshape(-1) for p in parts])
        wg = flat.size
        flat = np.concatenate([flat, wave_section(g("stage_w"), g("qhead_w"), np.zeros((256, 256), np.float32) if last else g("lhead_w"), cb, self.segs)])
        assert flat.size == self.lib.qv2x_codebook_level_floats(kc)
        blob = _dev(flat, self.dev)
        cb_off = wg - kc - kc * 256
        L.check(self.lib.qv2x_codebook_c2_f32(C.c_void_p(blob.data_ptr() + 4 * cb_off), kc,
                                              C.c_void_p(blob.data_ptr() + 4 * (wg - kc)), L.current_stream()),
                "qv2x_codebook_c2_f32")
        return blob

    def _padded(self, n, h, w, c, q):
        t = torch.empty((n, h + 2, w + 2, c), dtype=torch.int8, device=self.dev)
        t.fill_(int(q[1]) - 128)
        return t

    def _workspace(self, n: int) -> dict:
        if n in self._bufs:
            return self._bufs[n]
        b = {}
        h, w = self.ny, self.nx
        if self.encoder_kind == "second":
            from .engine_second import DeployedSecondEncoder
            self.second[n] = DeployedSecondEncoder(self.state, self.dev, agents=n, max_voxels=self.second_max_voxels, max_points=self.second_max_points)
            b["canvas"] = self.second[n].bev
        else:
            b["canvas"] = self._padded(n, h, w, 64, self.canvas_q)
        b["lvl"] = []
        for lvl, convs in enumerate(self.blocks):
            h, w = (h + 2 - 3) // self.strides[lvl] + 1, (w + 2 - 3) // self.strides[lvl] + 1
            zps = {c.out_q[1] for c in convs}
            if len(zps) != 1:
                raise NotImplementedError("conv outputs of one backbone level must share a zero point (post-ReLU: 0)")
            pair = [self._padded(n, h, w, convs[0].cout, convs[0].out_q) for _ in range(2)]
            b["lvl"].append((pair, h, w))
        (_, h0, w0) = b["lvl"][0]
        self.fh, self.fw = h0 * self.ups[0], w0 * self.ups[0]
        for lvl, (_, hl, wl) in enumerate(b["lvl"]):
            if (hl * self.ups[lvl], wl * self.ups[lvl]) != (self.fh, self.fw):
                raise ValueError(f"deblock {lvl} upsamples {hl}x{wl} by {self.ups[lvl]} to {hl * self.ups[lvl]}x{wl * self.ups[lvl]}, "
                                 f"level 0 gives {self.fh}x{self.fw}: the grid does not line up across backbone levels")
        cat = torch.empty((n, self.fh + 2, self.fw + 2, self.cat_channels), dtype=torch.int8, device=self.dev)
        c0 = 0
        for de in self.deblocks:
            cat[..., c0:c0 + de.cout] = int(de.out_q[1]) - 128
            c0 += de.cout
        b["cat"] = cat
        b["s0"] = self._padded(n, self.fh, self.fw, self.shrink0.cout, self.shrink0.out_q)
        b["s1"] = self._padded(n, self.fh, self.fw, self.shrink1.cout, self.shrink1.out_q)
        if self.compress:
            b["comp"] = [self._padded(n, self.fh, self.fw, c.cout, c.out_q) for c in self.comp]
        hw = self.fh * self.fw
        if self.has_codebook:
            b["codes"] = torch.empty((self.levels, n, hw), dtype=torch.uint8, device=self.dev)
        if self.two_stage_supported():
            if self._two_stage is None and self.encode_mode == "two_stage":
                self._build_two_stage()
            b["enc_list"] = torch.zeros(3 * n * hw, dtype=torch.int32, device=self.dev)
            b["enc_counters"] = torch.zeros(4, dtype=torch.int32, device=self.dev)
        if not self.has_codebook or self.heads_single is not None:
            b["feats"] = torch.empty((n, hw, 256), dtype=torch.float32, device=self.dev)
        self._bufs[n] = b
        return b

    def _conv(self, layer: _ConvLayer, x, n, h, w, out, out_ctotal=None, out_c0=0):
        d = L.ConvDesc()
        d.n, d.h, d.w, d.cin_total, d.stride, d.cout = n, h, w, x.shape[-1], layer.stride, layer.cout
        d.ngroups = len(layer.groups)
        for i, (c0, c, zx) in enumerate(layer.groups):
            d.group_c0[i], d.group_c[i], d.group_zx[i] = c0, c, zx
        d.out_ctotal = out.shape[-1] if out_ctotal is None else out_ctotal
        d.out_c0, d.relu = out_c0, 1
        d.out_delta, d.out_zp = layer.out_q[0], float(layer.out_q[1])
        if self.use_wide_conv and self.lib.qv2x_conv3x3_i8_wide_ok(C.byref(d)):
            if layer.w_wide is None:
                layer.w_wide = torch.empty_like(layer.w)
                L.check(self.lib.qv2x_conv3x3_i8_pack_wide(C.byref(d), L.ptr(layer.w), L.ptr(layer.w_wide), L.current_stream()), layer.name)
            L.check(self.lib.qv2x_conv3x3_i8_wide(C.byref(d), L.ptr(x), L.ptr(layer.w_wide), L.ptr(layer.scale), L.ptr(layer.corr),
                                                  L.ptr(layer.aw), L.ptr(layer.bias), L.ptr(out), L.current_stream()), layer.name)
            return
        L.check(self.lib.qv2x_conv3x3_i8(C.byref(d), L.ptr(x), L.ptr(layer.w), L.ptr(layer.scale), L.ptr(layer.corr),
                                         L.ptr(layer.aw), L.ptr(layer.bias), L.ptr(out), L.current_stream()), layer.name)

    def _chain(self, ch: _ChainLayers, x, n, h, w, out):
        d = L.ChainDesc()
        d.n, d.in_h, d.in_w = n, h, w
        d.h, d.w = out.shape[1] - 2, out.shape[2] - 2
        d.depth, d.stride0, d.relu = len(ch.convs), ch.stride0, 1
        for i, c in enumerate(ch.convs):
            d.out_delta[i], d.out_zp[i] = c.out_q[0], float(c.out_q[1])
        L.check(self.lib.qv2x_conv3x3_i8_chain64(C.byref(d), L.ptr(x), L.ptr(ch.w), L.ptr(ch.scale), L.ptr(ch.corr), L.ptr(ch.aw),
                                                 L.ptr(ch.bias), L.ptr(out), L.current_stream()), ch.name)

    def _deconv_desc(self, de: _DeconvLayer, n, h, w, out, out_c0):
        d = L.DeconvDesc()
        d.n, d.h, d.w, d.cin, d.cout, d.s = n, h, w, de.cin, de.cout, de.s
        d.in_zx, d.in_delta = int(de.in_q[1]), float(de.in_q[0])
        d.out_ctotal, d.out_c0, d.relu = out.shape[-1], out_c0, 1
        d.out_delta, d.out_zp = de.out_q[0], float(de.out_q[1])
        d.out_h, d.out_w = out.shape[1] - 2, out.shape[2] - 2
        return d

    def _deconv(self, de: _DeconvLayer, x, n, h, w, out, out_c0):
        d = self._deconv_desc(de, n, h, w, out, out_c0)
        L.check(self.lib.qv2x_deconv_i8(C.byref(d), L.ptr(x), L.ptr(de.w), L.ptr(de.bias), L.ptr(out), L.current_stream()), de.name)

    def _deconv_batch(self, items, n):
        k = len(items)
        descs = (L.DeconvDesc * k)(*[self._deconv_desc(de, n, h, w, out, c0) for (de, x, h, w, out, c0) in items])
        arr = lambda ts: (C.c_void_p * k)(*[t.data_ptr() for t in ts])
        L.check(self.lib.qv2x_deconv_i8_batch(descs, k, arr([it[1] for it in items]), arr([it[0].w for it in items]),
                                              arr([it[0].bias for it in items]), arr([it[4] for it in items]), L.current_stream()),
                "qv2x_deconv_i8_batch")

    def _run_heads(self, hd: _Heads, rows, nb, hw):
        out = torch.empty((nb, hd.cout, self.fh, self.fw), dtype=torch.float32, device=self.dev)
        L.check(self.lib.qv2x_heads_f32(L.ptr(rows), nb * hw, hw, hd.cout, hd.cout_pad, L.ptr(hd.w), L.ptr(hd.bias),
                                        L.ptr(hd.da), L.ptr(hd.za), L.ptr(out), L.current_stream()), "qv2x_heads_f32")
        return out

    def conv_plan(self, n_agents: int):
        b = self._workspace(n_agents)
        use_chains = self.use_chains and n_agents <= self.chain_max_agents
        key = ("plan", use_chains)
        if key in b:
            return b[key]
        plan = []
        x, h, w, c0 = b["canvas"], self.ny, self.nx, 0
        for lvl, convs in enumerate(self.blocks):
            pair, ho, wo = b["lvl"][lvl]
            macs = [n_agents * ho * wo * layer.cout * layer.w.shape[1] for layer in convs]
            if use_chains and self.chains[lvl] is not None:
                out = pair[(len(convs) - 1) % 2]
                plan.append(("chain", self.chains[lvl], x, h, w, out, 0, sum(macs)))
                x, h, w = out, ho, wo
            else:
                for i, layer in enumerate(convs):
                    out = pair[i % 2]
                    plan.append(("conv", layer, x, h, w, out, 0, macs[i]))
                    x, h, w = out, ho, wo
            de = self.deblocks[lvl]
            plan.append(("deconv", de, x, h, w, b["cat"], c0, n_agents * h * w * de.cin * de.cout * de.s * de.s))
            c0 += de.cout
        hw = n_agents * self.fh * self.fw
        plan.append(("conv", self.shrink0, b["cat"], self.fh, self.fw, b["s0"], 0, hw * self.shrink0.cout * self.shrink0.w.shape[1]))
        plan.append(("conv", self.shrink1, b["s0"], self.fh, self.fw, b["s1"], 0, hw * self.shrink1.cout * self.shrink1.w.shape[1]))
        if self.compress:
            x = b["s1"]
            for c, out in zip(self.comp, b["comp"]):
                plan.append(("conv", c, x, self.fh, self.fw, out, 0, hw * c.cout * c.w.shape[1]))
                x = out
        b[key] = plan
        return plan

    def run_plan(self, n_agents: int, only=None, taps: Optional[dict] = None):
        pending = []

        def flush():
            if len(pending) == 1:
                de, x, h, w, out, c0 = pending[0]
                self._deconv(de, x, n_agents, h, w, out, c0)
            elif pending:
                self._deconv_batch(pending, n_agents)
            pending.clear()

        for (kind, layer, x, h, w, out, c0, _) in self.conv_plan(n_agents):
            if only is not None and not only(kind, layer):
                continue
            if kind == "chain":
                self._chain(layer, x, n_agents, h, w, out)
                if taps is not None:
                    taps[layer.name] = out.clone()
            elif kind == "conv":
                if layer is self.shrink0:
                    flush()
                self._conv(layer, x, n_agents, h, w, out)
                if taps is not None:
                    taps[layer.name] = out.clone()
            else:
                pending.append((layer, x, h, w, out, c0))
                if not self.batch_deconvs:
                    flush()
        flush()

    def pillars_to_canvas(self, inputs: dict, n_agents: int, resident: bool = False):
        b = self._workspace(n_agents)
        st = L.current_stream()
        vf = inputs["voxel_features"].contiguous()
        co = inputs["voxel_coords"].to(torch.int32).contiguous()
        npnt = inputs["voxel_num_points"].to(torch.int32).contiguous()
        if self.encoder_kind == "second":
            return self.second[n_agents]({"voxel_features": vf, "voxel_coords": co, "voxel_num_points": npnt})
        if vf.dtype != torch.float32 or vf.dim() != 3 or tuple(vf.shape[1:]) != (32, 4):
            raise ValueError("voxel_features must be float32 [M, 32, 4]")
        canvas = b["canvas"]
        capturing = torch.cuda.is_current_stream_capturing()
        if not resident and b.get("fill_less_graphs", False):
            raise L.Qv2xError("pillars_to_canvas(resident=False) on a workspace whose captured graphs rely on the clean resident canvas: "
                              "use resident=True + clear_pillars, or another DeployedModel")
        if not (resident and b.get("canvas_clean", False)):
            L.check(self.lib.qv2x_fill_i8(L.ptr(canvas), canvas.numel(), int(self.pfn.z2) - 128, st), "qv2x_fill_i8")
        elif capturing:
            b["fill_less_graphs"] = True
        b["canvas_clean"] = False
        L.check(self.lib.qv2x_pfn_scatter_i8(L.ptr(vf), L.ptr(co), L.ptr(npnt), vf.shape[0], 32, C.byref(self.pfn),
                                             L.ptr(canvas), n_agents, self.ny, self.nx, st), "qv2x_pfn_scatter_i8")
        return canvas

    def _restore_canvas(self, n_agents: int):
        b = self._workspace(n_agents)
        if self.encoder_kind != "second" and not torch.cuda.is_current_stream_capturing():
            L.check(self.lib.qv2x_fill_i8(L.ptr(b["canvas"]), b["canvas"].numel(), int(self.pfn.z2) - 128, L.current_stream()), "qv2x_fill_i8")
            b["canvas_clean"] = True

    def clear_pillars(self, inputs: dict, n_agents: int):
        if self.encoder_kind == "second":
            return
        b = self._workspace(n_agents)
        co = inputs["voxel_coords"].to(torch.int32).contiguous()
        L.check(self.lib.qv2x_pfn_unscatter_i8(L.ptr(co), co.shape[0], int(self.pfn.z2) - 128, L.ptr(b["canvas"]), n_agents, self.ny, self.nx,
                                               L.current_stream()), "qv2x_pfn_unscatter_i8")
        b["canvas_clean"] = True

    def encode_codes(self, n_agents: int, out: Optional[torch.Tensor] = None):
        b = self._workspace(n_agents)
        codes = b["codes"] if out is None else out
        if codes.dtype != torch.uint8 or not codes.is_contiguous() or codes.numel() != self.levels * n_agents * self.fh * self.fw:
            raise ValueError("encode_codes: out must be a contiguous uint8 tensor [levels, n_agents, H*W]")
        d = L.EncodeDesc()
        d.n, d.h, d.w, d.levels, d.kc, d.segs = n_agents, self.fh, self.fw, self.enc_levels, self.kc, self.segs
        d.in_zx, d.in_delta = int(self.shrink1.out_q[1]), float(self.shrink1.out_q[0])
        two_stage = self.encode_mode == "two_stage" and self.encode_form == "auto"
        if two_stage and self._two_stage is None:
            self._refuse_during_capture("encode_mode 'two_stage'")
            self._build_two_stage()
            two_stage = self.encode_mode == "two_stage"
        if self.encode_mode == "collapsed":
            if self.segs != 1 or self.kc > 128:
                raise NotImplementedError("encode_mode 'collapsed': seg_num 1 and dict_size <= 128 (the exact encode takes the rest)")
            if self._collapsed is None:
                self._refuse_during_capture("encode_mode 'collapsed'")
                self._collapsed = tuple(_dev(t, self.dev) for t in collapse_encoder(self.state, self.enc_levels, d.in_delta, d.in_zx))
            gp, bias, tab = self._collapsed
            L.check(self.lib.qv2x_codebook_encode_collapsed_f32(C.byref(d), L.ptr(b["s1"]), L.ptr(gp), L.ptr(bias), L.ptr(tab), L.ptr(codes),
                                                                L.current_stream()), "qv2x_codebook_encode_collapsed_f32")
            return codes
        if two_stage:
            return self._encode_two_stage(d, b, codes)
        if self.encode_mode not in ("exact", "two_stage"):
            raise ValueError(f"encode_mode {self.encode_mode!r}: 'exact' (every cell through the reference's op order), 'two_stage' (the same "
                             "indices: exact integer candidates, the chain only where the bound cannot decide) or 'collapsed' (opt-in, approximate)")
        if self.encode_form == "wave":
            L.check(self.lib.qv2x_codebook_encode_wave_f32(C.byref(d), L.ptr(b["s1"]), None, self.level_ptrs, L.ptr(codes),
                                                           L.current_stream()), "qv2x_codebook_encode_wave_f32")
            return codes
        L.check(self.lib.qv2x_codebook_encode_f32(C.byref(d), L.ptr(b["s1"]), self.level_ptrs, L.ptr(codes),
                                                  L.current_stream()), "qv2x_codebook_encode_f32")
        return codes

    def two_stage_supported(self) -> bool:
        if not self.has_codebook or self.enc_levels > 3 or self.kc > 256:
            return False
        return bool(self.kc % 32 == 0 if self.segs == 1 else self.segs == 2 and self.kc % 64 == 0)

    def _refuse_during_capture(self, what: str):
        if torch.cuda.is_current_stream_capturing():
            raise L.Qv2xError(f"{what}: its operands are built on the host and uploaded -- not inside a HIP-graph capture; encode once "
                              "in this mode before capturing")

    def _build_two_stage(self):
        if not self.two_stage_supported():
            raise NotImplementedError("encode_mode 'two_stage': seg_num 1 | 2, dict_size <= 256, up to three levels (encode_mode 'exact' takes the rest)")
        from .encode_two_stage import candidate_tables
        try:
            t = candidate_tables(self.state, self.enc_levels, float(self.shrink1.out_q[0]), int(self.shrink1.out_q[1]), self.segs)
            k = np.arange(t["bias"].shape[0], dtype=np.int64) % self.kc
            pf = int(t["pack"])
            packed = (pf * t["bias"] + k).astype(np.float64)
            if not np.array_equal(packed.astype(np.int64), pf * t["bias"] + k):
                raise ValueError("two-stage encode: packed scores not exact in float64")
            self._two_stage = (_dev(t["gpack"], self.dev), _dev(packed, self.dev), _dev(t["tables"], self.dev),
                               (C.c_float * (3 * self.enc_levels))(*[float(v) for v in t["tau"].reshape(-1)]), t)
        except Exception as e:
            self.encode_mode, self.two_stage_refused = "exact", str(e) or type(e).__name__

    def candidate_entry(self) -> str:
        from .encode_two_stage import CANDIDATE_ENTRY, pack_factor
        return CANDIDATE_ENTRY[pack_factor(self.segs, self.kc)]

    def _encode_two_stage(self, d, b, codes):
        gp, bias, tab, tau, _ = self._two_stage
        name = self.candidate_entry()
        L.check(getattr(self.lib, name)(C.byref(d), L.ptr(b["s1"]), L.ptr(gp), L.ptr(bias), L.ptr(tab), tau, L.ptr(codes),
                                        L.ptr(b["enc_list"]), L.ptr(b["enc_counters"]), L.current_stream()), name)
        L.check(self.lib.qv2x_codebook_encode_listed_f32(C.byref(d), L.ptr(b["s1"]), self.level_ptrs, L.ptr(b["enc_list"]), L.ptr(b["enc_counters"]),
                                                         L.ptr(codes), L.current_stream()), "qv2x_codebook_encode_listed_f32")
        return codes

    def encode_refine_stats(self, n_agents: int) -> dict:
        if not (self.encode_mode == "two_stage" and self.encode_form == "auto") or "enc_counters" not in self._bufs.get(n_agents, {}):
            raise L.Qv2xError(f"encode_refine_stats({n_agents}): no two-stage encode of {n_agents} frames here (encode_mode "
                              f"{self.encode_mode!r}, encode_form {self.encode_form!r}, workspaces {sorted(self._bufs)})")
        c = self._bufs[n_agents]["enc_counters"].cpu().numpy().astype(np.int64)
        cells = n_agents * self.fh * self.fw
        return {"cells": cells, "refined": int(c[0]), "refined_fraction": float(c[0]) / cells, "first_flagged_at_level": [int(v) for v in c[1:1 + self.enc_levels]]}

    def wire_shape(self):
        self._workspace(1)
        return self.levels, self.fh * self.fw

    def encode_into(self, inputs: dict, frames: int, codes_out: torch.Tensor):
        self.pillars_to_canvas(inputs, frames, resident=True)
        try:
            self.run_plan(frames)
            self.clear_pillars(inputs, frames)
        except BaseException:
            self._restore_canvas(frames)
            raise
        return self.encode_codes(frames, out=codes_out)

    def pairwise_from_poses(self, gathered: torch.Tensor, world: int, agent_stride: int, pose_offset: int, max_cav: int, out: torch.Tensor):
        L.check(self.lib.qv2x_pairwise_from_poses_f64(L.ptr(gathered), world, agent_stride, pose_offset, max_cav, L.ptr(out),
                                                      L.current_stream()), "qv2x_pairwise_from_poses_f64")

    def pairwise_frames_from_poses(self, gathered: torch.Tensor, world: int, agent_stride: int, pose_offset: int, frames: int, frame_stride: int,
                                   max_cav: int, out: torch.Tensor):
        L.check(self.lib.qv2x_pairwise_from_poses_batch_f64(L.ptr(gathered), world, agent_stride, pose_offset, frames, frame_stride, max_cav,
                                                            L.ptr(out), L.current_stream()), "qv2x_pairwise_from_poses_batch_f64")

    def fuse_frames_and_heads(self, gathered: torch.Tensor, agent_stride: int, level_stride: int, frame_stride: int, pairwise: torch.Tensor,
                              n_agents: int, ego: int, own_codes: Optional[torch.Tensor], frames: int) -> dict:
        lens = [n_agents] * frames
        form = self._post_form(lens, None, own_codes is not None and frame_stride == self.fh * self.fw)
        return self._post(form, L.ptr(gathered), agent_stride, level_stride, None, pairwise, [f * frame_stride for f in range(frames)], lens, ego,
                          own_codes, frames)

    def band_shape(self):
        self._workspace(1)
        return self.heads.cout, self.fh, self.fw

    def head_wire_supported(self, wire: str) -> bool:
        if wire not in L.WIRES:
            raise ValueError(f"wire: one of {sorted(L.WIRES)}, got {wire!r}")
        return wire == "f32" or bool((self.heads.da_np > 0).all())

    def fuse_frames_and_heads_band(self, gathered: torch.Tensor, agent_stride: int, level_stride: int, frame_stride: int, pairwise: torch.Tensor,
                                   n_agents: int, ego: int, frames: int, y0: int, y1: int, out_slab: torch.Tensor, wire: str = "f32"):
        if not self.head_wire_supported(wire):
            raise L.Qv2xError("band wire 'u8': a head without an output quantizer has no codes to send")
        hd, n_cells, esz = self.heads, (y1 - y0) * self.fw, (1 if wire == "u8" else 4)
        if not 0 <= y0 <= y1 <= self.fh:
            raise ValueError(f"band rows [{y0}, {y1}) outside the map's {self.fh} rows")
        if out_slab.dtype != torch.uint8 or out_slab.numel() < frames * hd.cout * n_cells * esz:
            raise ValueError("out_slab: u8, at least frames * cout * band cells * element size bytes")
        if n_cells == 0:
            return
        one_launch = self.band_one_launch
        if one_launch is None:
            one_launch = frames * n_cells // 32 >= self.fuse_heads_min_tiles and n_agents <= self._one_launch_agents()
        rows = None
        if not one_launch:
            key = (frames, n_cells)
            if self._band_rows is None or self._band_rows[0] != key:
                self._band_rows = (key, torch.empty((frames, n_cells, 256), dtype=torch.float32, device=self.dev))
            rows = self._band_rows[1]
        lut = L.ptr(self.lut) if self.has_codebook else None
        lb = L.ptr(self.lut_bias) if self.has_codebook else None
        base, st = out_slab.data_ptr(), L.current_stream()
        for s0 in range(0, frames, 64):
            s1 = min(frames, s0 + 64)
            d = self._fuse_desc(agent_stride, level_stride, pairwise[s0], n_agents, ego)
            offs = (C.c_int64 * (s1 - s0))(*[f * frame_stride for f in range(s0, s1)])
            cnts = (C.c_int32 * (s1 - s0))(*([n_agents] * (s1 - s0)))
            out = C.c_void_p(base + s0 * hd.cout * n_cells * esz)
            if one_launch:
                L.check(self.lib.qv2x_fuse_heads_band(C.byref(d), s1 - s0, offs, cnts, L.ptr(gathered), lut, lb, None, L.ptr(pairwise[s0]),
                                                      y0 * self.fw, n_cells, hd.cout, hd.cout_pad, L.ptr(hd.w), L.ptr(hd.bias), L.ptr(hd.da),
                                                      L.ptr(hd.za), L.WIRES[wire], L.ptr(hd.da_np), out, None, st), "qv2x_fuse_heads_band")
            else:
                L.check(self.lib.qv2x_fuse_att_band_f32(C.byref(d), s1 - s0, offs, cnts, L.ptr(gathered), lut, lb, None, L.ptr(pairwise[s0]),
                                                        y0 * self.fw, n_cells, L.ptr(rows[s0]), st), "qv2x_fuse_att_band_f32")
                L.check(self.lib.qv2x_heads_band(L.ptr(rows[s0]), s1 - s0, n_cells, hd.cout, hd.cout_pad, L.ptr(hd.w), L.ptr(hd.bias),
                                                 L.ptr(hd.da), L.ptr(hd.za), L.WIRES[wire], L.ptr(hd.da_np), out, st), "qv2x_heads_band")

    def assemble_bands(self, gathered_slabs: torch.Tensor, world: int, frames: int, wire: str, out: torch.Tensor):
        hd = self.heads
        L.check(self.lib.qv2x_assemble_bands(L.ptr(gathered_slabs), world, gathered_slabs.shape[1], frames, hd.cout, self.fh, self.fw, L.WIRES[wire],
                                             L.ptr(hd.da), L.ptr(hd.za), L.ptr(out), L.current_stream()), "qv2x_assemble_bands")

    def band_output(self, preds: torch.Tensor, own_codes: Optional[torch.Tensor], frames: int) -> dict:
        out = split_heads(preds, self.heads.splits)
        if own_codes is not None:
            out.update(self.single_preds(own_codes, frames))
        return out

    def encode_agents(self, inputs: dict, n_agents: int, taps: Optional[dict] = None):
        b = self._workspace(n_agents)
        canvas = self.pillars_to_canvas(inputs, n_agents, resident=True)
        try:
            self.run_plan(n_agents, taps=taps)
            if taps is not None:
                taps["canvas"], taps["cat"] = canvas.clone(), b["cat"]
            self.clear_pillars(inputs, n_agents)
        except BaseException:
            self._restore_canvas(n_agents)
            raise
        if taps is not None:
            taps[self.shrink0.name], taps[self.shrink1.name] = b["s0"], b["s1"]
        if taps is not None and self.compress:
            for c, out in zip(self.comp, b["comp"]):
                taps[c.name] = out
        return self.encode_codes(n_agents) if self.has_codebook else (b["comp"][-1] if self.compress else b["s1"])

    def decode_rows(self, codes, n_rows_total):
        out = torch.empty((n_rows_total, 256), dtype=torch.float32, device=self.dev)
        L.check(self.lib.qv2x_decode_lut_f32(L.ptr(codes), n_rows_total, self.levels, self.kc, L.ptr(self.lut),
                                             L.ptr(self.lut_bias), L.ptr(out), L.current_stream()), "qv2x_decode_lut_f32")
        return out

    def _fuse_desc(self, agent_stride, level_stride, pairwise_b, n, ego):
        d = L.FuseDesc()
        d.agents, d.h, d.w = n, self.fh, self.fw
        d.levels, d.kc = (self.levels, self.kc) if self.has_codebook else (1, 1)
        d.max_cav, d.ego = pairwise_b.shape[0], ego
        d.code_agent_stride, d.code_level_stride = agent_stride, level_stride
        d.h_metres, d.w_metres, d.discrete_ratio = self.hm, self.wm, self.ratio
        d.fusion = self.fusion
        return d

    def fuse(self, codes_ptr, agent_stride, level_stride, feats, pairwise_b, n, out, ego=0):
        d = self._fuse_desc(agent_stride, level_stride, pairwise_b, n, ego)
        lut = L.ptr(self.lut) if self.has_codebook else None
        lb = L.ptr(self.lut_bias) if self.has_codebook else None
        L.check(self.lib.qv2x_fuse_att_f32(C.byref(d), codes_ptr, lut, lb, L.ptr(feats) if feats is not None else None,
                                           L.ptr(pairwise_b), L.ptr(out), L.current_stream()), "qv2x_fuse_att_f32")

    def fuse_scenes(self, codes_ptr, agent_stride, level_stride, feats, pairwise, offsets, counts, out, ego=0):
        for s0 in range(0, len(counts), 64):
            s1 = min(len(counts), s0 + 64)
            d = self._fuse_desc(agent_stride, level_stride, pairwise[s0], max(counts[s0:s1]), ego)
            offs = (C.c_int64 * (s1 - s0))(*offsets[s0:s1])
            cnts = (C.c_int32 * (s1 - s0))(*counts[s0:s1])
            lut = L.ptr(self.lut) if self.has_codebook else None
            lb = L.ptr(self.lut_bias) if self.has_codebook else None
            L.check(self.lib.qv2x_fuse_att_batch_f32(C.byref(d), s1 - s0, offs, cnts, codes_ptr, lut, lb,
                                                     L.ptr(feats) if feats is not None else None, L.ptr(pairwise[s0]), L.ptr(out[s0]),
                                                     L.current_stream()), "qv2x_fuse_att_batch_f32")

    def _self_transforms_are_identity(self, pairwise: torch.Tensor) -> bool:
        if pairwise.is_cuda:
            if torch.cuda.is_current_stream_capturing():
                return True
            ref = getattr(self, "_ident_ref", None)
            if ref is not None and ref[0]() is pairwise and ref[1] == pairwise._version:
                return ref[2]
            t00 = pairwise[:, 0, 0].cpu()
        else:
            t00 = pairwise[:, 0, 0]
        ok = bool((t00 == torch.eye(4, dtype=t00.dtype)).all())
        if pairwise.is_cuda:
            import weakref
            self._ident_ref = (weakref.ref(pairwise), pairwise._version, ok)
        return ok

    def _one_launch_agents(self) -> int:
        batched = self.has_codebook and self.levels == 3
        return self.fuse_heads_max_agents if batched else min(self.fuse_heads_max_agents, 1)

    def _table_heads_out(self, codes, n: int) -> dict:
        tab, tb, da, za, c0, c1 = self.table_heads
        hw = self.fh * self.fw
        preds = torch.empty((n, c0, self.fh, self.fw), dtype=torch.float32, device=self.dev)
        sp = torch.empty((n, c1, self.fh, self.fw), dtype=torch.float32, device=self.dev) if c1 else None
        L.check(self.lib.qv2x_table_heads_f32(L.ptr(codes), n * hw, hw, self.levels, self.kc, c0, c1, L.ptr(tab), L.ptr(tb), L.ptr(da), L.ptr(za),
                                              L.ptr(preds), L.ptr(sp) if sp is not None else None, L.current_stream()), "qv2x_table_heads_f32")
        out = split_heads(preds, self.heads.splits)
        if sp is not None:
            out.update(split_heads(sp, self.heads_single.splits, "_single"))
        return out

    def fuse_heads_scenes(self, codes_ptr, agent_stride, level_stride, feats, pairwise, offsets, counts, ego=0, fused_tap=None):
        hd, hw = self.heads, self.fh * self.fw
        out = torch.empty((len(counts), hd.cout, self.fh, self.fw), dtype=torch.float32, device=self.dev)
        for s0 in range(0, len(counts), 64):
            s1 = min(len(counts), s0 + 64)
            d = self._fuse_desc(agent_stride, level_stride, pairwise[s0], max(counts[s0:s1]), ego)
            offs = (C.c_int64 * (s1 - s0))(*offsets[s0:s1])
            cnts = (C.c_int32 * (s1 - s0))(*counts[s0:s1])
            lut = L.ptr(self.lut) if self.has_codebook else None
            lb = L.ptr(self.lut_bias) if self.has_codebook else None
            L.check(self.lib.qv2x_fuse_heads_batch_f32(C.byref(d), s1 - s0, offs, cnts, codes_ptr, lut, lb,
                                                       L.ptr(feats) if feats is not None else None, L.ptr(pairwise[s0]),
                                                       hd.cout, hd.cout_pad, L.ptr(hd.w), L.ptr(hd.bias), L.ptr(hd.da), L.ptr(hd.za), L.ptr(out[s0]),
                                                       L.ptr(fused_tap[s0]) if fused_tap is not None else None, L.current_stream()),
                    "qv2x_fuse_heads_batch_f32")
        return out

    def _post_form(self, lens: List[int], taps: Optional[dict], identity) -> str:
        if (taps is None and self.table_heads is not None and self.single_agent_tables and all(n == 1 for n in lens)
                and (identity() if callable(identity) else identity)):
            return "tables"
        if taps is None and len(lens) * self.fh * self.fw // 32 >= self.fuse_heads_min_tiles and max(lens) <= self._one_launch_agents():
            return "one_launch"
        return "fused"

    def _post(self, form: str, codes_ptr, agent_stride, level_stride, feats, pairwise, offsets, lens: List[int], ego: int,
              own: Optional[torch.Tensor], n_own: int, taps: Optional[dict] = None) -> dict:
        if form == "tables":
            return self._table_heads_out(own, len(lens))
        hw, nb = self.fh * self.fw, len(lens)
        single = self.heads_single is not None and own is not None
        sp = None
        if form == "one_launch":
            preds = self.fuse_heads_scenes(codes_ptr, agent_stride, level_stride, feats, pairwise, offsets, lens, ego)
            if single:
                sp = self._decode_heads_single(own, n_own)
        else:
            fused = torch.empty((nb, hw, 256), dtype=torch.float32, device=self.dev)
            self.fuse_scenes(codes_ptr, agent_stride, level_stride, feats, pairwise, offsets, lens, fused, ego)
            if single:
                preds, sp = self._heads_pair(fused, nb, own, n_own)
            else:
                preds = self._run_heads(self.heads, fused, nb, hw)
            if taps is not None:
                taps["fused"] = fused
        if self.heads_single is not None and sp is None and feats is not None:
            sp = self._run_heads(self.heads_single, feats, sum(lens), hw)
        out = split_heads(preds, self.heads.splits)
        if sp is not None:
            out.update(split_heads(sp, self.heads_single.splits, "_single"))
        return out

    def fuse_and_heads(self, codes, agent_stride, level_stride, pairwise_b, n_agents, ego=0) -> dict:
        return self.fuse_heads_and_single(codes, agent_stride, level_stride, pairwise_b, n_agents, ego, None, 0)

    def _decode_heads_single(self, codes, n_agents: int):
        hw = self.fh * self.fw
        hd = self.heads_single
        sp = torch.empty((n_agents, hd.cout, self.fh, self.fw), dtype=torch.float32, device=self.dev)
        if self.single_by_tables:
            tab, tb = hd.lut_tables
            L.check(self.lib.qv2x_single_heads_lut_f32(L.ptr(codes), n_agents * hw, hw, self.levels, self.kc, hd.cout, L.ptr(tab), L.ptr(tb),
                                                       L.ptr(hd.da), L.ptr(hd.za), L.ptr(sp), L.current_stream()), "qv2x_single_heads_lut_f32")
            return sp
        if self.single_by_global_tables:
            tab, tb = hd.lut_tables
            L.check(self.lib.qv2x_table_heads_f32(L.ptr(codes), n_agents * hw, hw, self.levels, self.kc, hd.cout, 0, L.ptr(tab), L.ptr(tb),
                                                  L.ptr(hd.da), L.ptr(hd.za), L.ptr(sp), None, L.current_stream()), "qv2x_table_heads_f32")
            return sp
        L.check(self.lib.qv2x_decode_heads_f32(L.ptr(codes), n_agents * hw, hw, self.levels, self.kc, L.ptr(self.lut), L.ptr(self.lut_bias),
                                               hd.cout, hd.cout_pad, L.ptr(hd.w), L.ptr(hd.bias), L.ptr(hd.da), L.ptr(hd.za),
                                               L.ptr(sp), L.current_stream()), "qv2x_decode_heads_f32")
        return sp

    def _heads_pair(self, fused, nb, codes, n_agents):
        hw = self.fh * self.fw
        hd, hs = self.heads, self.heads_single
        if self.single_by_tables or self.single_by_global_tables:
            return self._run_heads(hd, fused, nb, hw), self._decode_heads_single(codes, n_agents)
        preds = torch.empty((nb, hd.cout, self.fh, self.fw), dtype=torch.float32, device=self.dev)
        sp = torch.empty((n_agents, hs.cout, self.fh, self.fw), dtype=torch.float32, device=self.dev)
        L.check(self.lib.qv2x_heads_pair_f32(L.ptr(fused), nb * hw, hw, hd.cout, hd.cout_pad, L.ptr(hd.w), L.ptr(hd.bias), L.ptr(hd.da),
                                             L.ptr(hd.za), L.ptr(preds), L.ptr(codes), n_agents * hw, self.levels, self.kc,
                                             L.ptr(self.lut), L.ptr(self.lut_bias), hs.cout, hs.cout_pad, L.ptr(hs.w), L.ptr(hs.bias),
                                             L.ptr(hs.da), L.ptr(hs.za), L.ptr(sp), L.current_stream()), "qv2x_heads_pair_f32")
        return preds, sp

    def fuse_heads_and_single(self, codes, agent_stride, level_stride, pairwise_b, n_agents, ego, own_codes, n_own: int = 1) -> dict:
        pairwise = pairwise_b.to(torch.float64).contiguous()[None]
        return self._post("fused", L.ptr(codes), agent_stride, level_stride, None, pairwise, [0], [n_agents], ego, own_codes, n_own)

    def single_preds(self, codes, n_agents: int) -> dict:
        if self.heads_single is None:
            return {}
        return split_heads(self._decode_heads_single(codes, n_agents), self.heads_single.splits, "_single")

    def _shared_features(self, shrinker_out, n_total: int):
        q = self.final.out_q
        feats = self._workspace(n_total)["feats"]
        L.check(self.lib.qv2x_dequant_i8_f32(L.ptr(shrinker_out), n_total, self.fh, self.fw, 256, int(q[1]), float(q[0]), L.ptr(feats),
                                             L.current_stream()), "qv2x_dequant_i8_f32")
        return feats

    @torch.no_grad()
    def forward(self, data_dict: dict, taps: Optional[dict] = None) -> dict:
        agents = data_dict["agent_modality_list"]
        n_total = len(agents)
        if any(a != "m1" for a in agents):
            raise NotImplementedError("deployed path: every agent is the LiDAR modality 'm1' (a heterogeneous model deploys as DeployedHeterModel)")
        enc = self.encode_agents(data_dict["inputs_m1"], n_total, taps)
        return self.finish(enc, n_total, data_dict, taps)

    @torch.no_grad()
    def finish(self, enc, n_total: int, data_dict: dict, taps: Optional[dict] = None) -> dict:
        pairwise, lens = scene_layout(data_dict, n_total)
        hw = self.fh * self.fw
        feats = None if self.has_codebook else self._shared_features(enc, n_total)
        form = self._post_form(lens, taps, lambda: self._self_transforms_are_identity(data_dict["pairwise_t_matrix"]))
        if form != "tables" and not pairwise.is_cuda:
            if torch.cuda.is_current_stream_capturing():
                raise ValueError("pairwise_t_matrix on the host cannot be uploaded during HIP-graph capture: pass a device tensor")
            pairwise = pairwise.to(self.dev)
        starts = [sum(lens[:bi]) for bi in range(len(lens))]
        if self.has_codebook:
            out = self._post(form, L.ptr(enc), hw, n_total * hw, None, pairwise, [st * hw for st in starts], lens, 0, enc, n_total, taps)
        else:
            out = self._post(form, None, 0, 0, feats, pairwise, [st * hw * 256 for st in starts], lens, 0, None, n_total, taps)
        if taps is not None:
            taps["codes"] = enc if self.has_codebook else None
            taps["features"] = feats
        return out

    def capture(self, data_dict: dict):
        return capture_forward(self, data_dict)


class DeployedHeterModel(nn.Module):

    def __init__(self, states: Dict[str, Dict[str, np.ndarray]], ego_modality: Optional[str] = None, device="cuda", **kw):
        super().__init__()
        if not states:
            raise ValueError("DeployedHeterModel: no modality")
        self.engines = {m: DeployedModel(st, device=device, **kw) for m, st in states.items()}
        self.main = self.engines[ego_modality if ego_modality in self.engines else next(iter(self.engines))]
        for m, e in self.engines.items():
            e._workspace(1)
            if not e.has_codebook:
                raise NotImplementedError("deployed heterogeneous path: codebook models (the code planes are what the modalities share)")
            if (e.fh, e.fw, e.levels, e.kc) != (self.main.fh, self.main.fw, self.main.levels, self.main.kc):
                raise ValueError(f"modality {m}: feature map {e.fh} x {e.fw} / codebook {e.levels} x {e.kc} differs from the ego modality's")
        self.dev = self.main.dev
        self._slots: Dict[tuple, Dict[str, torch.Tensor]] = {}

    @torch.no_grad()
    def forward(self, data_dict: dict, taps: Optional[dict] = None) -> dict:
        agents = list(data_dict["agent_modality_list"])
        enc = assemble_heter_codes("DeployedHeterModel", self.engines, self._slots, agents, data_dict,
                                   lambda eng, inputs, k, mt: eng.encode_agents(inputs, k, mt), taps)
        return self.main.finish(enc, len(agents), data_dict, taps)

    def capture(self, data_dict: dict):
        return capture_forward(self, data_dict)


def deploy_heter(qt_model, device="cuda", **kw) -> DeployedHeterModel:
    model = qt_model.model if hasattr(qt_model, "model") else qt_model
    states = {m: export_ptq_state(qt_model, modality=m) for m in model.modality_name_list}
    return DeployedHeterModel(states, ego_modality=getattr(model, "ego_modality", None), device=device, **kw)


def deploy(qt_model=None, state: Optional[Dict[str, np.ndarray]] = None, path: Optional[str] = None,
           device="cuda", **kw) -> DeployedModel:
    if state is None:
        if path is not None:
            state = load_ptq_state(path)
        elif any(hasattr(m, "weight_quantizer") for m in qt_model.modules()):
            inner = qt_model.model if hasattr(qt_model, "model") else qt_model
            if len(getattr(inner, "modality_name_list", ["m1"])) > 1:
                if hasattr(inner, "pyramid_backbone"):
                    from .engine_pyramid import deploy_heter_pyramid
                    return deploy_heter_pyramid(qt_model, device=device)
                return deploy_heter(qt_model, device=device, **kw)
            state = export_ptq_state(qt_model)
        elif hasattr(qt_model, "pyramid_backbone"):
            from .engine_pyramid_fp32 import export_fp32_pyramid_state
            state = export_fp32_pyramid_state(qt_model)
        else:
            from .engine_fp32 import export_fp32_state
            state = export_fp32_state(qt_model)
    if str(state.get("meta/mode", "w8a8")) == "fp32":
        if str(state.get("meta/fusion_method", "att")) == "pyramid":
            from .engine_pyramid_fp32 import DeployedPyramidFp32Model
            return DeployedPyramidFp32Model(state, device=device, **kw)
        from .engine_fp32 import DeployedFp32Model
        return DeployedFp32Model(state, device=device, **kw)
    if str(state.get("meta/fusion_method", "att")) == "pyramid":
        from .engine_pyramid import DeployedPyramidModel
        return DeployedPyramidModel(state, device=device, **kw)
    return DeployedModel(state, device=device, **kw)
```

### quantv2x_amd/lib.py

```python
from __future__ import annotations

import ctypes as C
import os

_HERE = os.path.dirname(os.path.abspath(__file__))
LIB_PATH = os.path.join(_HERE, "libqv2x.so")
MAX_GROUPS = 4
ABI_VERSION = 9

SYMBOLS = [
    "qv2x_last_error", "qv2x_version", "qv2x_fill_i8", "qv2x_pfn_scatter_i8", "qv2x_pfn_unscatter_i8", "qv2x_conv3x3_i8",
    "qv2x_conv3x3_i8_wide_ok", "qv2x_conv3x3_i8_pack_wide", "qv2x_conv3x3_i8_wide", "qv2x_conv3x3_i8_chain64",
    "qv2x_deconv_i8", "qv2x_deconv_i8_batch", "qv2x_codebook_level_floats", "qv2x_codebook_c2_f32", "qv2x_codebook_encode_f32", "qv2x_codebook_encode_wave_f32", "qv2x_fuse_att_f32", "qv2x_fuse_att_batch_f32", "qv2x_fuse_heads_batch_f32",
    "qv2x_decode_lut_f32", "qv2x_single_heads_lut_f32", "qv2x_table_heads_f32", "qv2x_dequant_i8_f32", "qv2x_heads_f32", "qv2x_decode_heads_f32", "qv2x_heads_pair_f32", "qv2x_voxelize_workspace_bytes", "qv2x_voxelize_f32",
    "qv2x_postprocess_workspace_bytes", "qv2x_postprocess_f32", "qv2x_postprocess_late_workspace_bytes", "qv2x_postprocess_late_f32",
    "qv2x_conv3x3_f32", "qv2x_deconv_f32", "qv2x_pfn_scatter_f32", "qv2x_codebook_encode_f32in",
    "qv2x_pyramid_weighted_fuse_f32", "qv2x_pyramid_weighted_fuse_i8", "qv2x_conv1x1_i8", "qv2x_gconv3x3_i8", "qv2x_conv3x3_i8_res",
    "qv2x_deconv_f32in", "qv2x_codebook_decode_f32", "qv2x_occ_score_i8",
    "qv2x_codebook64_level_floats", "qv2x_codebook64_c2_f32", "qv2x_codebook_encode64_f32", "qv2x_codebook_encode64_f32in",
    "qv2x_add_relu_f32", "qv2x_occ_sigmoid_f32", "qv2x_pyramid_weighted_fuse_f32p", "qv2x_bottleneck_i8",
    "qv2x_comm_unique_id", "qv2x_comm_init", "qv2x_comm_destroy", "qv2x_allgather_codes", "qv2x_pairwise_from_poses_f64", "qv2x_pairwise_from_poses_batch_f64",
    "qv2x_codebook_encode_collapsed_f32", "qv2x_codebook_encode_candidates_i8", "qv2x_codebook_encode_candidates_seg_i8", "qv2x_codebook_encode_listed_f32", "qv2x_mean_vfe_f32", "qv2x_sp_index_scatter", "qv2x_sp_out_sites_workspace_bytes", "qv2x_sp_out_sites", "qv2x_sp_rulebook", "qv2x_sp_conv_f32in", "qv2x_sp_conv_i8", "qv2x_sp_to_bev_i8",
    "qv2x_fuse_att_band_f32", "qv2x_heads_band", "qv2x_fuse_heads_band", "qv2x_assemble_bands",
    "qv2x_voxelize_batch_workspace_bytes", "qv2x_voxelize_batch_f32", "qv2x_postprocess_batch_workspace_bytes", "qv2x_postprocess_batch_f32",
    "qv2x_eval_workspace_bytes", "qv2x_eval_tp_fp_f32", "qv2x_gt_boxes_f32",
]
WIRES = {"f32": 0, "u8": 1}
COMM_ID_BYTES = 128


class PfnParams(C.Structure):
    _fields_ = [("w", C.c_float * 640), ("b", C.c_float * 64),
                ("d1", C.c_float), ("z1", C.c_float), ("d2", C.c_float), ("z2", C.c_float),
                ("vox", C.c_float * 3), ("off", C.c_float * 3)]


class ConvDesc(C.Structure):
    _fields_ = [("n", C.c_int32), ("h", C.c_int32), ("w", C.c_int32), ("cin_total", C.c_int32),
                ("stride", C.c_int32), ("cout", C.c_int32), ("ngroups", C.c_int32),
                ("group_c0", C.c_int32 * MAX_GROUPS), ("group_c", C.c_int32 * MAX_GROUPS),
                ("group_zx", C.c_int32 * MAX_GROUPS),
                ("out_ctotal", C.c_int32), ("out_c0", C.c_int32), ("relu", C.c_int32),
                ("out_delta", C.c_float), ("out_zp", C.c_float)]


class ChainDesc(C.Structure):
    _fields_ = [("n", C.c_int32), ("h", C.c_int32), ("w", C.c_int32), ("in_h", C.c_int32), ("in_w", C.c_int32),
                ("depth", C.c_int32), ("stride0", C.c_int32), ("relu", C.c_int32),
                ("out_delta", C.c_float * 4), ("out_zp", C.c_float * 4)]


class DeconvDesc(C.Structure):
    _fields_ = [("n", C.c_int32), ("h", C.c_int32), ("w", C.c_int32), ("cin", C.c_int32), ("cout", C.c_int32),
                ("s", C.c_int32), ("in_zx", C.c_int32), ("in_delta", C.c_float),
                ("out_ctotal", C.c_int32), ("out_c0", C.c_int32), ("relu", C.c_int32),
                ("out_delta", C.c_float), ("out_zp", C.c_float), ("out_h", C.c_int32), ("out_w", C.c_int32)]


class F32ConvDesc(C.Structure):
    _fields_ = [("n", C.c_int32), ("h", C.c_int32), ("w", C.c_int32), ("cin_total", C.c_int32), ("cin0", C.c_int32), ("cin", C.c_int32),
                ("stride", C.c_int32), ("cout", C.c_int32), ("out_ctotal", C.c_int32), ("out_c0", C.c_int32), ("relu", C.c_int32)]


class Conv1x1Desc(C.Structure):
    _fields_ = [("n", C.c_int32), ("h", C.c_int32), ("w", C.c_int32), ("cin", C.c_int32), ("cout", C.c_int32), ("stride", C.c_int32),
                ("mode", C.c_int32), ("relu", C.c_int32), ("out_ctotal", C.c_int32), ("out_c0", C.c_int32),
                ("out_delta", C.c_float), ("out_zp", C.c_float), ("res_zx", C.c_int32), ("res_delta", C.c_float)]


class BottleneckDesc(C.Structure):
    _fields_ = [("n", C.c_int32), ("h", C.c_int32), ("w", C.c_int32), ("planes", C.c_int32), ("width", C.c_int32), ("cg", C.c_int32),
                ("in_zx", C.c_int32), ("in_delta", C.c_float), ("delta1", C.c_float), ("zp1", C.c_float), ("delta2", C.c_float), ("zp2", C.c_float),
                ("out_delta", C.c_float), ("out_zp", C.c_float)]


class GconvDesc(C.Structure):
    _fields_ = [("n", C.c_int32), ("h", C.c_int32), ("w", C.c_int32), ("c", C.c_int32), ("cg", C.c_int32), ("stride", C.c_int32),
                ("relu", C.c_int32), ("out_delta", C.c_float), ("out_zp", C.c_float)]


class SpconvDesc(C.Structure):
    _fields_ = [("subm", C.c_int32), ("k", C.c_int32 * 3), ("s", C.c_int32 * 3), ("p", C.c_int32 * 3),
                ("in_shape", C.c_int32 * 3), ("out_shape", C.c_int32 * 3), ("agents", C.c_int32), ("cin", C.c_int32), ("cout", C.c_int32),
                ("cap_in", C.c_int32), ("cap_out", C.c_int32), ("out_delta", C.c_float), ("out_zp", C.c_float)]


class OccDesc(C.Structure):
    _fields_ = [("n", C.c_int32), ("h", C.c_int32), ("w", C.c_int32), ("c", C.c_int32), ("aw", C.c_int32), ("corr", C.c_int32),
                ("scale", C.c_float), ("bias", C.c_float), ("out_delta", C.c_float), ("out_zp", C.c_float)]


class EncodeDesc(C.Structure):
    _fields_ = [("n", C.c_int32), ("h", C.c_int32), ("w", C.c_int32), ("levels", C.c_int32), ("kc", C.c_int32),
                ("in_zx", C.c_int32), ("in_delta", C.c_float), ("segs", C.c_int32)]


class FuseDesc(C.Structure):
    _fields_ = [("agents", C.c_int32), ("h", C.c_int32), ("w", C.c_int32), ("levels", C.c_int32), ("kc", C.c_int32),
                ("max_cav", C.c_int32), ("ego", C.c_int32),
                ("code_agent_stride", C.c_int64), ("code_level_stride", C.c_int64),
                ("h_metres", C.c_double), ("w_metres", C.c_double), ("discrete_ratio", C.c_double), ("fusion", C.c_int32)]


class PostprocessDesc(C.Structure):
    _fields_ = [("h", C.c_int32), ("w", C.c_int32), ("anchors_per_cell", C.c_int32), ("num_bins", C.c_int32),
                ("score_threshold", C.c_float), ("nms_threshold", C.c_float), ("dir_offset", C.c_float),
                ("range", C.c_float * 6), ("transform", C.c_float * 16), ("max_boxes", C.c_int32),
                ("num_classes", C.c_int32), ("range_xy_only", C.c_int32),
                ("max_extent", C.c_float), ("z_min", C.c_float), ("z_max", C.c_float)]


class EvalDesc(C.Structure):
    _fields_ = [("frames", C.c_int32), ("det_cap", C.c_int32), ("gt_cap", C.c_int32), ("n_classes", C.c_int32), ("n_ranges", C.c_int32),
                ("n_thresholds", C.c_int32), ("ranges", (C.c_float * 2) * 4), ("thresholds", C.c_float * 4)]


class GtDesc(C.Structure):
    _fields_ = [("frames", C.c_int32), ("agents", C.c_int32), ("obj_cap", C.c_int32), ("gt_cap", C.c_int32), ("row_floats", C.c_int32),
                ("order", C.c_int32), ("mode", C.c_int32), ("range_xy_only", C.c_int32), ("range", C.c_float * 6), ("iou_threshold", C.c_float)]


class Qv2xError(RuntimeError):
    pass


_lib = None


def load() -> C.CDLL:
    global _lib
    if _lib is not None:
        return _lib
    if not os.path.exists(LIB_PATH):
        raise Qv2xError(f"{LIB_PATH} is missing: build it with `python -c 'import __graft_entry__ as g; g.build()'` "
                        "(hipcc --offload-arch=gfx950).  There is no CPU fallback for the deployed path.")
    lib = C.CDLL(LIB_PATH)
    missing = [s for s in SYMBOLS if not hasattr(lib, s)]
    if missing:
        raise Qv2xError(f"libqv2x.so does not export {missing}")
    vp = C.c_void_p
    lib.qv2x_last_error.restype = C.c_char_p
    lib.qv2x_version.restype = C.c_int
    if lib.qv2x_version() != ABI_VERSION:
        raise Qv2xError(f"libqv2x.so has ABI {lib.qv2x_version()}, this binding mirrors ABI {ABI_VERSION} (include/qv2x.h): rebuild the library")
    lib.qv2x_fill_i8.argtypes = [vp, C.c_int64, C.c_int, vp]
    lib.qv2x_pfn_scatter_i8.argtypes = [vp, vp, vp, C.c_int, C.c_int, C.POINTER(PfnParams), vp, C.c_int, C.c_int, C.c_int, vp]
    lib.qv2x_pfn_unscatter_i8.argtypes = [vp, C.c_int, C.c_int, vp, C.c_int, C.c_int, C.c_int, vp]
    lib.qv2x_conv3x3_i8.argtypes = [C.POINTER(ConvDesc), vp, vp, vp, vp, vp, vp, vp, vp]
    lib.qv2x_conv3x3_i8_wide.argtypes = [C.POINTER(ConvDesc), vp, vp, vp, vp, vp, vp, vp, vp]
    lib.qv2x_conv3x3_i8_chain64.argtypes = [C.POINTER(ChainDesc), vp, vp, vp, vp, vp, vp, vp, vp]
    lib.qv2x_conv3x3_i8_pack_wide.argtypes = [C.POINTER(ConvDesc), vp, vp, vp]
    lib.qv2x_conv3x3_i8_wide_ok.argtypes = [C.POINTER(ConvDesc)]
    lib.qv2x_deconv_i8.argtypes = [C.POINTER(DeconvDesc), vp, vp, vp, vp, vp]
    lib.qv2x_deconv_i8_batch.argtypes = [C.POINTER(DeconvDesc), C.c_int, C.POINTER(vp), C.POINTER(vp), C.POINTER(vp), C.POINTER(vp), vp]
    lib.qv2x_codebook_level_floats.argtypes = [C.c_int]
    lib.qv2x_codebook_level_floats.restype = C.c_int64
    lib.qv2x_codebook_c2_f32.argtypes = [vp, C.c_int, vp, vp]
    lib.qv2x_codebook_encode_f32.argtypes = [C.POINTER(EncodeDesc), vp, C.POINTER(vp), vp, vp]
    lib.qv2x_codebook_encode_wave_f32.argtypes = [C.POINTER(EncodeDesc), vp, vp, C.POINTER(vp), vp, vp]
    lib.qv2x_fuse_att_f32.argtypes = [C.POINTER(FuseDesc), vp, vp, vp, vp, vp, vp, vp]
    lib.qv2x_fuse_att_batch_f32.argtypes = [C.POINTER(FuseDesc), C.c_int, C.POINTER(C.c_int64), C.POINTER(C.c_int32), vp, vp, vp, vp, vp, vp, vp]
    lib.qv2x_decode_lut_f32.argtypes = [vp, C.c_int, C.c_int, C.c_int, vp, vp, vp, vp]
    lib.qv2x_fuse_heads_batch_f32.argtypes = [C.POINTER(FuseDesc), C.c_int, C.POINTER(C.c_int64), C.POINTER(C.c_int32), vp, vp, vp, vp, vp,
                                              C.c_int, C.c_int, vp, vp, vp, vp, vp, vp, vp]
    lib.qv2x_heads_f32.argtypes = [vp, C.c_int, C.c_int, C.c_int, C.c_int, vp, vp, vp, vp, vp, vp]
    lib.qv2x_decode_heads_f32.argtypes = [vp, C.c_int, C.c_int, C.c_int, C.c_int, vp, vp, C.c_int, C.c_int, vp, vp, vp, vp, vp, vp]
    lib.qv2x_table_heads_f32.argtypes = [vp, C.c_int, C.c_int, C.c_int, C.c_int, C.c_int, C.c_int, vp, vp, vp, vp, vp, vp, vp]
    lib.qv2x_single_heads_lut_f32.argtypes = [vp, C.c_int, C.c_int, C.c_int, C.c_int, C.c_int, vp, vp, vp, vp, vp, vp]
    lib.qv2x_heads_pair_f32.argtypes = [vp, C.c_int, C.c_int, C.c_int, C.c_int, vp, vp, vp, vp, vp,
                                        vp, C.c_int, C.c_int, C.c_int, vp, vp, C.c_int, C.c_int, vp, vp, vp, vp, vp, vp]
    lib.qv2x_dequant_i8_f32.argtypes = [vp, C.c_int, C.c_int, C.c_int, C.c_int, C.c_int, C.c_float, vp, vp]
    lib.qv2x_codebook_encode_collapsed_f32.argtypes = [C.POINTER(EncodeDesc), vp, vp, vp, vp, vp, vp]
    lib.qv2x_codebook_encode_candidates_i8.argtypes = [C.POINTER(EncodeDesc), vp, vp, vp, vp, C.POINTER(C.c_float), vp, vp, vp, vp]
    lib.qv2x_codebook_encode_candidates_seg_i8.argtypes = [C.POINTER(EncodeDesc), vp, vp, vp, vp, C.POINTER(C.c_float), vp, vp, vp, vp]
    lib.qv2x_codebook_encode_listed_f32.argtypes = [C.POINTER(EncodeDesc), vp, C.POINTER(vp), vp, vp, vp, vp]
    lib.qv2x_mean_vfe_f32.argtypes = [vp, vp, vp, C.c_int, C.c_int, vp, vp]
    lib.qv2x_sp_index_scatter.argtypes = [vp, vp, C.c_int, C.c_int, C.c_int, C.c_int, C.c_int, vp, C.c_int, vp]
    lib.qv2x_sp_out_sites_workspace_bytes.argtypes = [C.POINTER(SpconvDesc)]
    lib.qv2x_sp_out_sites_workspace_bytes.restype = C.c_int64
    lib.qv2x_sp_out_sites.argtypes = [C.POINTER(SpconvDesc), vp, vp, vp, vp, vp, vp, C.c_int64, vp]
    lib.qv2x_sp_rulebook.argtypes = [C.POINTER(SpconvDesc), vp, vp, vp, vp, vp]
    lib.qv2x_sp_conv_f32in.argtypes = [C.POINTER(SpconvDesc), vp, vp, vp, vp, vp, vp, vp, vp]
    lib.qv2x_sp_conv_i8.argtypes = [C.POINTER(SpconvDesc), vp, vp, vp, vp, vp, vp, vp, vp, vp, vp, vp]
    lib.qv2x_sp_to_bev_i8.argtypes = [vp, vp, vp, C.c_int, C.c_int, C.c_int, C.c_int, C.c_int, C.c_int, C.c_int, C.c_int, vp, vp]
    lib.qv2x_voxelize_workspace_bytes.argtypes = [C.c_int]
    lib.qv2x_voxelize_workspace_bytes.restype = C.c_int64
    lib.qv2x_voxelize_f32.argtypes = [vp, C.c_int, C.POINTER(C.c_float), C.POINTER(C.c_float), C.c_int, C.c_int, C.c_int,
                                      vp, C.c_int64, vp, vp, vp, vp, vp]
    lib.qv2x_voxelize_batch_workspace_bytes.argtypes = [C.c_int, C.POINTER(C.c_int32)]
    lib.qv2x_voxelize_batch_workspace_bytes.restype = C.c_int64
    lib.qv2x_voxelize_batch_f32.argtypes = [C.POINTER(vp), C.POINTER(C.c_int32), C.c_int, C.POINTER(C.c_float), C.POINTER(C.c_float),
                                            C.c_int, C.c_int, C.c_int, vp, C.c_int64, vp, vp, vp, vp, vp]
    lib.qv2x_postprocess_batch_workspace_bytes.argtypes = [C.POINTER(PostprocessDesc), C.c_int]
    lib.qv2x_postprocess_batch_workspace_bytes.restype = C.c_int64
    lib.qv2x_postprocess_batch_f32.argtypes = [C.POINTER(PostprocessDesc), C.c_int, vp, C.c_int64, vp, C.c_int64, vp, C.c_int64, vp, vp,
                                               vp, C.c_int64, vp, vp, vp, vp, vp]
    lib.qv2x_eval_workspace_bytes.argtypes = [C.POINTER(EvalDesc)]
    lib.qv2x_eval_workspace_bytes.restype = C.c_int64
    lib.qv2x_eval_tp_fp_f32.argtypes = [C.POINTER(EvalDesc), vp, vp, vp, vp, vp, vp, vp, vp, C.c_int64, vp, vp, vp, vp, vp, vp]
    lib.qv2x_gt_boxes_f32.argtypes = [C.POINTER(GtDesc), vp, vp, vp, vp, vp, vp, vp, vp, vp, vp, vp]
    lib.qv2x_postprocess_workspace_bytes.argtypes = [C.POINTER(PostprocessDesc)]
    lib.qv2x_postprocess_workspace_bytes.restype = C.c_int64
    lib.qv2x_postprocess_f32.argtypes = [C.POINTER(PostprocessDesc), vp, vp, vp, vp, vp, C.c_int64, vp, vp, vp, vp, vp]
    lib.qv2x_postprocess_late_workspace_bytes.argtypes = [C.POINTER(PostprocessDesc), C.c_int]
    lib.qv2x_postprocess_late_workspace_bytes.restype = C.c_int64
    lib.qv2x_postprocess_late_f32.argtypes = [C.POINTER(PostprocessDesc), C.c_int, C.POINTER(vp), C.POINTER(vp), C.POINTER(vp), C.POINTER(vp),
                                              C.POINTER(C.c_float), vp, C.c_int64, vp, vp, vp, vp, vp]
    lib.qv2x_conv3x3_f32.argtypes = [C.POINTER(F32ConvDesc), vp, vp, vp, vp, vp]
    lib.qv2x_deconv_f32.argtypes = [C.POINTER(F32ConvDesc), vp, vp, vp, vp, vp]
    lib.qv2x_pfn_scatter_f32.argtypes = [vp, vp, vp, C.c_int, C.c_int, C.POINTER(C.c_float), C.POINTER(C.c_float), C.POINTER(C.c_float),
                                         C.POINTER(C.c_float), vp, C.c_int, C.c_int, C.c_int, vp]
    lib.qv2x_codebook_encode_f32in.argtypes = [C.POINTER(EncodeDesc), vp, C.POINTER(vp), vp, vp]
    lib.qv2x_pyramid_weighted_fuse_f32.argtypes = [C.POINTER(FuseDesc), C.c_int, vp, vp, vp, vp, vp]
    lib.qv2x_pyramid_weighted_fuse_i8.argtypes = [C.POINTER(FuseDesc), C.c_int, vp, C.c_int, C.c_float, vp, vp, vp, vp]
    lib.qv2x_conv1x1_i8.argtypes = [C.POINTER(Conv1x1Desc), vp, vp, vp, vp, vp, vp, vp, vp, vp]
    lib.qv2x_gconv3x3_i8.argtypes = [C.POINTER(GconvDesc), vp, vp, vp, vp, vp, vp, vp, vp]
    lib.qv2x_conv3x3_i8_res.argtypes = [C.POINTER(ConvDesc), vp, vp, vp, vp, vp, vp, C.c_int, vp, C.c_int, C.c_float, vp, vp]
    lib.qv2x_deconv_f32in.argtypes = [C.POINTER(DeconvDesc), vp, vp, vp, vp, vp]
    lib.qv2x_codebook_decode_f32.argtypes = [vp, C.c_int64, C.c_int64, C.c_int, C.c_int, C.c_int, C.c_int, C.c_int, vp, vp, vp, vp]
    lib.qv2x_occ_score_i8.argtypes = [C.POINTER(OccDesc), vp, vp, vp, vp, vp, vp]
    lib.qv2x_codebook64_level_floats.argtypes = [C.c_int]
    lib.qv2x_codebook64_level_floats.restype = C.c_int64
    lib.qv2x_codebook64_c2_f32.argtypes = [vp, C.c_int, vp, vp]
    lib.qv2x_codebook_encode64_f32.argtypes = [C.POINTER(EncodeDesc), C.c_int, vp, C.POINTER(vp), vp, vp]
    lib.qv2x_codebook_encode64_f32in.argtypes = [C.POINTER(EncodeDesc), C.c_int, vp, C.POINTER(vp), vp, vp]
    lib.qv2x_add_relu_f32.argtypes = [vp, vp, vp, C.c_int64, vp]
    lib.qv2x_occ_sigmoid_f32.argtypes = [vp, C.c_int, C.c_int, C.c_int, C.c_int, vp, vp, vp]
    lib.qv2x_pyramid_weighted_fuse_f32p.argtypes = [C.POINTER(FuseDesc), C.c_int, vp, vp, vp, vp, vp]
    lib.qv2x_bottleneck_i8.argtypes = [C.POINTER(BottleneckDesc), vp, C.POINTER(vp), C.POINTER(vp), C.POINTER(vp), C.POINTER(vp), C.POINTER(vp), vp, vp]
    lib.qv2x_comm_unique_id.argtypes = [vp]
    lib.qv2x_comm_init.argtypes = [vp, C.c_int, C.c_int, C.POINTER(vp)]
    lib.qv2x_comm_destroy.argtypes = [vp]
    lib.qv2x_allgather_codes.argtypes = [vp, vp, vp, C.c_int64, vp]
    lib.qv2x_pairwise_from_poses_f64.argtypes = [vp, C.c_int, C.c_int64, C.c_int64, C.c_int, vp, vp]
    lib.qv2x_pairwise_from_poses_batch_f64.argtypes = [vp, C.c_int, C.c_int64, C.c_int64, C.c_int, C.c_int64, C.c_int, vp, vp]
    lib.qv2x_fuse_att_band_f32.argtypes = [C.POINTER(FuseDesc), C.c_int, C.POINTER(C.c_int64), C.POINTER(C.c_int32), vp, vp, vp, vp, vp,
                                           C.c_int64, C.c_int64, vp, vp]
    lib.qv2x_heads_band.argtypes = [vp, C.c_int, C.c_int64, C.c_int, C.c_int, vp, vp, vp, vp, C.c_int, vp, vp, vp]
    lib.qv2x_fuse_heads_band.argtypes = [C.POINTER(FuseDesc), C.c_int, C.POINTER(C.c_int64), C.POINTER(C.c_int32), vp, vp, vp, vp, vp,
                                         C.c_int64, C.c_int64, C.c_int, C.c_int, vp, vp, vp, vp, C.c_int, vp, vp, vp, vp]
    lib.qv2x_assemble_bands.argtypes = [vp, C.c_int, C.c_int64, C.c_int, C.c_int, C.c_int, C.c_int, C.c_int, vp, vp, vp, vp]
    for s in SYMBOLS:
        if s not in ("qv2x_last_error", "qv2x_codebook_level_floats", "qv2x_codebook64_level_floats", "qv2x_voxelize_workspace_bytes", "qv2x_postprocess_workspace_bytes",
                     "qv2x_postprocess_late_workspace_bytes", "qv2x_sp_out_sites_workspace_bytes", "qv2x_voxelize_batch_workspace_bytes",
                     "qv2x_postprocess_batch_workspace_bytes", "qv2x_eval_workspace_bytes"):
            getattr(lib, s).restype = C.c_int
    _lib = lib
    return lib


def check(rc: int, what: str = "") -> None:
    if rc != 0:
        msg = load().qv2x_last_error().decode(errors="replace")
        raise Qv2xError(f"{what or 'libqv2x'} failed with {rc}: {msg}")


def ptr(t) -> C.c_void_p:
    if t is None:
        return C.c_void_p(0)
    if hasattr(t, "data_ptr"):
        return C.c_void_p(t.data_ptr())
    return C.c_void_p(t.ctypes.data)


def current_stream() -> C.c_void_p:
    import torch
    return C.c_void_p(torch.cuda.current_stream().cuda_stream)
```

Measured before the change: 6879.

## Broadcast pillar points via DPP and fold encode counter reset into unscatter

The 16-lane PFN scatter kernel now spreads a pillar's up-to-32 points across the 16 lanes (two float4 per lane) and broadcasts each point with DPP row-broadcast, replacing the serial per-point global loads. It also prefetches point counts one round ahead, and the kernel is picked automatically by max_points. Separately, zeroing the two-stage encode counters moves into the canvas unscatter kernel, which removes one tiny kernel launch per frame. This adds new ABI entry points and a compile-time unrolled slot loop that may raise register pressure.

```diff
diff --git a/include/qv2x.h b/include/qv2x.h
--- a/include/qv2x.h
+++ b/include/qv2x.h
@@ -41,7 +41,13 @@
 int qv2x_pfn_scatter_i8(const float* voxel_features, const int32_t* voxel_coords, const int32_t* voxel_num_points,
                         int M, int max_points, const qv2x_pfn_params* params ,
                         int8_t* canvas, int N, int ny, int nx, void* stream);
+int qv2x_pfn_scatter_form_i8(const float* voxel_features, const int32_t* voxel_coords, const int32_t* voxel_num_points,
+                             int M, int max_points, const qv2x_pfn_params* params ,
+                             int8_t* canvas, int N, int ny, int nx, int lanes, void* stream);
+int qv2x_pfn_fetch_slot(int sub, int half, int num_points, int max_points);
 int qv2x_pfn_unscatter_i8(const int32_t* voxel_coords, int M, int value, int8_t* canvas, int N, int ny, int nx, void* stream);
+int qv2x_pfn_unscatter_reset_i8(const int32_t* voxel_coords, int M, int value, int8_t* canvas, int N, int ny, int nx,
+                                uint32_t* counters, int n_counters, void* stream);
 
 typedef struct {
     int32_t n, h, w, cin_total, stride, cout;
@@ -112,6 +118,12 @@
 int qv2x_codebook_encode_candidates_seg_i8(const qv2x_encode_desc* desc , const int8_t* in, const int8_t* g_limbs, const double* bias_packed,
                                            const int32_t* tables, const float* tau , uint8_t* codes, uint32_t* list, uint32_t* counters,
                                            void* stream);
+int qv2x_codebook_encode_candidates_cleared_i8(const qv2x_encode_desc* desc , const int8_t* in, const int8_t* g_limbs,
+                                               const double* bias_packed, const int32_t* tables, const float* tau , uint8_t* codes,
+                                               uint32_t* list, uint32_t* counters, void* stream);
+int qv2x_codebook_encode_candidates_seg_cleared_i8(const qv2x_encode_desc* desc , const int8_t* in, const int8_t* g_limbs,
+                                                   const double* bias_packed, const int32_t* tables, const float* tau , uint8_t* codes,
+                                                   uint32_t* list, uint32_t* counters, void* stream);
 
 typedef struct {
     int32_t agents, h, w, levels, kc;
diff --git a/quantv2x_amd/csrc/codebook_encode_cand.hip b/quantv2x_amd/csrc/codebook_encode_cand.hip
--- a/quantv2x_amd/csrc/codebook_encode_cand.hip
+++ b/quantv2x_amd/csrc/codebook_encode_cand.hip
@@ -206,7 +206,7 @@
 
 template <int PACK, int MAX_SEGS>
 int candidates(const char* me, const qv2x_encode_desc* d, const int8_t* in, const int8_t* g_limbs, const double* bias_packed, const int32_t* tables,
-               const float* tau, uint8_t* codes, uint32_t* list, uint32_t* counters, void* stream) {
+               const float* tau, uint8_t* codes, uint32_t* list, uint32_t* counters, void* stream, bool clear = true) {
     if (!d || !in || !g_limbs || !bias_packed || !tau || !codes || !list || !counters) return fail(QV2X_EINVAL, "%s: null pointer", me);
     if (d->n <= 0 || d->h <= 0 || d->w <= 0 || d->levels < 1 || d->levels > 3) return fail(QV2X_EINVAL, "%s: 1..3 levels", me);
     const int segs = d->segs ? d->segs : 1;
@@ -226,7 +226,7 @@
     a.tbytes = (d->levels > 1 ? d->levels * (d->levels - 1) / 2 : 1) * a.ke * a.ke * 4;
     a.delta = d->in_delta;
     hipStream_t st = (hipStream_t)stream;
-    zero_counters_kernel<<<1, 64, 0, st>>>(counters);
+    if (clear) zero_counters_kernel<<<1, 64, 0, st>>>(counters);
     int dev = 0, cus = 256, v = 0;
     if (hipGetDevice(&dev) == hipSuccess && hipDeviceGetAttribute(&v, hipDeviceAttributeMultiprocessorCount, dev) == hipSuccess && v > 0) cus = v;
     const bool large = a.M >= 4 * cus * 32 * (segs == 2 ? 3 : 4) * 2;
@@ -249,3 +249,15 @@
                                                       void* stream) {
     return qv2x::candidates<256, 2>("qv2x_codebook_encode_candidates_seg_i8", d, in, g_limbs, bias_packed, tables, tau, codes, list, counters, stream);
 }
+
+extern "C" int qv2x_codebook_encode_candidates_cleared_i8(const qv2x_encode_desc* d, const int8_t* in, const int8_t* g_limbs, const double* bias_packed,
+                                                          const int32_t* tables, const float* tau, uint8_t* codes, uint32_t* list, uint32_t* counters,
+                                                          void* stream) {
+    return qv2x::candidates<128, 1>("qv2x_codebook_encode_candidates_cleared_i8", d, in, g_limbs, bias_packed, tables, tau, codes, list, counters, stream, false);
+}
+
+extern "C" int qv2x_codebook_encode_candidates_seg_cleared_i8(const qv2x_encode_desc* d, const int8_t* in, const int8_t* g_limbs, const double* bias_packed,
+                                                              const int32_t* tables, const float* tau, uint8_t* codes, uint32_t* list, uint32_t* counters,
+                                                              void* stream) {
+    return qv2x::candidates<256, 2>("qv2x_codebook_encode_candidates_seg_cleared_i8", d, in, g_limbs, bias_packed, tables, tau, codes, list, counters, stream, false);
+}
diff --git a/quantv2x_amd/csrc/pfn_fetch.h b/quantv2x_amd/csrc/pfn_fetch.h
--- /dev/null
+++ b/quantv2x_amd/csrc/pfn_fetch.h
@@ -0,0 +1,28 @@
+#pragma once
+
+#ifdef __HIPCC__
+#define QV2X_HD __host__ __device__
+#else
+#define QV2X_HD
+#endif
+
+namespace qv2x {
+
+QV2X_HD inline int pfn_real(int np, int P) { return np < P ? np : P; }
+QV2X_HD inline bool pfn_fetch_second(int sub, int np, int P) {
+#ifdef PFN_FETCH_UNMASKED
+    return sub + 16 < P;
+#else
+    return sub + 16 < pfn_real(np, P);
+#endif
+}
+QV2X_HD inline int pfn_fetch_slot(int sub, int half, int np, int P) {
+    if (half) return sub + 16;
+#ifdef PFN_FETCH_UNMASKED
+    return sub < P ? sub : 0;
+#else
+    return sub < pfn_real(np, P) ? sub : 0;
+#endif
+}
+
+}
diff --git a/quantv2x_amd/csrc/pfn_scatter.hip b/quantv2x_amd/csrc/pfn_scatter.hip
--- a/quantv2x_amd/csrc/pfn_scatter.hip
+++ b/quantv2x_amd/csrc/pfn_scatter.hip
@@ -1,4 +1,6 @@
 #include "common.h"
+#include "pfn_fetch.h"
+#include <type_traits>
 
 namespace qv2x {
 
@@ -78,9 +80,20 @@
 }
 
 constexpr int PFN_R = 8;
-#ifndef PFN_NQ
-#define PFN_NQ 2
-#endif
+
+constexpr int PFN_SLOTS = 32;
+
+template <int L> __device__ __forceinline__ float pfn_row_bcast(float v) {
+    return __int_as_float(__builtin_amdgcn_update_dpp(0, __float_as_int(v), 0x150 + L, 0xf, 0xf, true));
+}
+template <int S, class F> __device__ __forceinline__ void pfn_slots(int real, F&& f) {
+    if constexpr (S < PFN_SLOTS) {
+        if (S < real) {
+            f(std::integral_constant<int, S>{});
+            pfn_slots<S + 1>(real, f);
+        }
+    }
+}
 
 __global__ __launch_bounds__(256, 4) void pfn_scatter16_kernel(const float4* __restrict__ vf, const int4* __restrict__ coords,
                                                             const int* __restrict__ npts, int M, int P,
@@ -108,32 +121,36 @@
     }
     const int mbase = blockIdx.x * (16 * rounds) + slot;
 
-    auto header = [&](int m, int4& c, int& np, float4 (&q)[PFN_NQ]) __attribute__((always_inline)) {
+    auto count = [&](int m) __attribute__((always_inline)) { return npts[m < M ? m : M - 1]; };
+    auto fetch = [&](int m, int np, int4& c, float4& qa, float4& qb) __attribute__((always_inline)) {
         const int mm = m < M ? m : M - 1;
         c = coords[mm];
-        np = npts[mm];
-#pragma unroll
-        for (int p = 0; p < PFN_NQ; ++p) q[p] = vf[(size_t)mm * P + (p < P ? p : P - 1)];
+        const float4* row = vf + (size_t)mm * P;
+        qa = row[pfn_fetch_slot(sub, 0, np, P)];
+        qb = make_float4(0.f, 0.f, 0.f, 0.f);
+        if (pfn_fetch_second(sub, np, P)) qb = row[pfn_fetch_slot(sub, 1, np, P)];
     };
     int4 c, cn;
-    int np, npn;
-    float4 q[PFN_NQ], qn[PFN_NQ];
-    header(mbase, c, np, q);
+    int np = count(mbase), npn = count(mbase + 16);
+    float4 qa, qb, qan, qbn;
+    fetch(mbase, np, c, qa, qb);
+    __builtin_amdgcn_s_waitcnt(0x0f70);
 #pragma unroll 1
     for (int r = 0; r < rounds; ++r) {
         const int m = mbase + r * 16;
-        if (r + 1 < rounds) header(m + 16, cn, npn, qn);
+        int npnn = 0;
+        if (r + 1 < rounds) {
+            fetch(m + 16, npn, cn, qan, qbn);
+            npnn = count(m + 32);
+        }
         if (m < M) {
-            const float4* pts = vf + (size_t)m * P;
             const int real = np < P ? np : P;
+            auto bx = [&](auto s) __attribute__((always_inline)) { return pfn_row_bcast<s.value & 15>(s.value < 16 ? qa.x : qb.x); };
+            auto by = [&](auto s) __attribute__((always_inline)) { return pfn_row_bcast<s.value & 15>(s.value < 16 ? qa.y : qb.y); };
+            auto bz = [&](auto s) __attribute__((always_inline)) { return pfn_row_bcast<s.value & 15>(s.value < 16 ? qa.z : qb.z); };
+            auto bw = [&](auto s) __attribute__((always_inline)) { return pfn_row_bcast<s.value & 15>(s.value < 16 ? qa.w : qb.w); };
             float sx = 0.f, sy = 0.f, sz = 0.f;
-#pragma unroll
-            for (int p = 0; p < PFN_NQ; ++p)
-                if (p < real) { sx += q[p].x; sy += q[p].y; sz += q[p].z; }
-            for (int p = PFN_NQ; p < real; ++p) {
-                const float4 t = pts[p];
-                sx += t.x; sy += t.y; sz += t.z;
-            }
+            pfn_slots<0>(real, [&](auto s) __attribute__((always_inline)) { sx += bx(s); sy += by(s); sz += bz(s); });
             const float n = (float)np;
             const float mx = sx / n, my = sy / n, mz = sz / n;
             const float cx = (float)c.w * prm.vox[0] + prm.off[0];
@@ -150,10 +167,7 @@
                     ymax[ch] = fmaxf(ymax[ch], acc + b[ch]);
                 }
             };
-#pragma unroll
-            for (int p = 0; p < PFN_NQ; ++p)
-                if (p < real) point(q[p]);
-            for (int p = PFN_NQ; p < real; ++p) point(pts[p]);
+            pfn_slots<0>(real, [&](auto s) __attribute__((always_inline)) { point(make_float4(bx(s), by(s), bz(s), bw(s))); });
             if (real < P) {
 #pragma unroll
                 for (int ch = 0; ch < 4; ++ch) ymax[ch] = fmaxf(ymax[ch], b[ch]);
@@ -166,14 +180,12 @@
                 *(unsigned*)(canvas + cell * 64 + sub * 4) = word;
             }
         }
-        c = cn; np = npn;
-#pragma unroll
-        for (int p = 0; p < PFN_NQ; ++p) q[p] = qn[p];
-    }
-}
-
-__global__ __launch_bounds__(256) void pfn_unscatter_kernel(const int4* __restrict__ coords, int M, int value4, int8_t* __restrict__ canvas,
-                                                            int N, int ny, int nx) {
+        c = cn; np = npn; npn = npnn;
+        qa = qan; qb = qbn;
+    }
+}
+
+__device__ __forceinline__ void pfn_unscatter_piece(const int4* __restrict__ coords, int M, int value4, int8_t* __restrict__ canvas, int N, int ny, int nx) {
     const long long id = (long long)blockIdx.x * 256 + threadIdx.x;
     const int m = (int)(id >> 2), piece = (int)(id & 3);
     if (m >= M) return;
@@ -184,6 +196,17 @@
     *(v4i*)(canvas + cell * 64 + piece * 16) = v;
 }
 
+__global__ __launch_bounds__(256) void pfn_unscatter_kernel(const int4* __restrict__ coords, int M, int value4, int8_t* __restrict__ canvas,
+                                                            int N, int ny, int nx) {
+    pfn_unscatter_piece(coords, M, value4, canvas, N, ny, nx);
+}
+
+__global__ __launch_bounds__(256) void pfn_unscatter_reset_kernel(const int4* __restrict__ coords, int M, int value4, int8_t* __restrict__ canvas,
+                                                                  int N, int ny, int nx, unsigned* __restrict__ counters, int words) {
+    if (blockIdx.x == 0 && (int)threadIdx.x < words) counters[threadIdx.x] = 0u;
+    pfn_unscatter_piece(coords, M, value4, canvas, N, ny, nx);
+}
+
 }
 
 extern "C" int qv2x_pfn_unscatter_i8(const int32_t* voxel_coords, int M, int value, int8_t* canvas, int N, int ny, int nx, void* stream) {
@@ -198,19 +221,52 @@
     return hip_check(hipGetLastError(), "qv2x_pfn_unscatter_i8 launch");
 }
 
+extern "C" int qv2x_pfn_unscatter_reset_i8(const int32_t* voxel_coords, int M, int value, int8_t* canvas, int N, int ny, int nx,
+                                           uint32_t* counters, int n_counters, void* stream) {
+    using namespace qv2x;
+    if (!counters || n_counters < 1 || n_counters > 256) return fail(QV2X_EINVAL, "qv2x_pfn_unscatter_reset_i8: 1 .. 256 counter words");
+    if (M < 0 || value < -128 || value > 127) return fail(QV2X_EINVAL, "qv2x_pfn_unscatter_reset_i8: bad sizes / value");
+    if (M > 0) {
+        if (!voxel_coords || !canvas) return fail(QV2X_EINVAL, "qv2x_pfn_unscatter_reset_i8: null pointer");
+        if (N <= 0 || ny <= 0 || nx <= 0) return fail(QV2X_EINVAL, "qv2x_pfn_unscatter_reset_i8: bad sizes / value");
+        if (((uintptr_t)voxel_coords & 15) || ((uintptr_t)canvas & 15)) return fail(QV2X_EALIGN, "qv2x_pfn_unscatter_reset_i8: coords / canvas must be 16-byte aligned");
+    }
+    if ((uintptr_t)counters & 3) return fail(QV2X_EALIGN, "qv2x_pfn_unscatter_reset_i8: counters must be 4-byte aligned");
+    const int b = value & 0xff, v4 = b | (b << 8) | (b << 16) | (b << 24);
+    const long long threads = (long long)M * 4;
+    const unsigned grid = threads ? (unsigned)((threads + 255) / 256) : 1u;
+    pfn_unscatter_reset_kernel<<<grid, 256, 0, (hipStream_t)stream>>>((const int4*)voxel_coords, M, v4, canvas, N, ny, nx, counters, n_counters);
+    return hip_check(hipGetLastError(), "qv2x_pfn_unscatter_reset_i8 launch");
+}
+
+extern "C" int qv2x_pfn_fetch_slot(int sub, int half, int num_points, int max_points) {
+    using namespace qv2x;
+    if (sub < 0 || sub > 15 || half < 0 || half > 1 || max_points <= 0 || max_points > PFN_SLOTS) return -1;
+    if (half && !pfn_fetch_second(sub, num_points, max_points)) return -1;
+    return pfn_fetch_slot(sub, half, num_points, max_points);
+}
+
 extern "C" int qv2x_pfn_scatter_i8(const float* voxel_features, const int32_t* voxel_coords, const int32_t* voxel_num_points,
                                    int M, int max_points, const qv2x_pfn_params* params, int8_t* canvas, int N, int ny, int nx,
                                    void* stream) {
-    using namespace qv2x;
+    return qv2x_pfn_scatter_form_i8(voxel_features, voxel_coords, voxel_num_points, M, max_points, params, canvas, N, ny, nx, 0, stream);
+}
+
+extern "C" int qv2x_pfn_scatter_form_i8(const float* voxel_features, const int32_t* voxel_coords, const int32_t* voxel_num_points,
+                                        int M, int max_points, const qv2x_pfn_params* params, int8_t* canvas, int N, int ny, int nx,
+                                        int lanes, void* stream) {
+    using namespace qv2x;
+    if (lanes != 0 && lanes != 16 && lanes != 64) return fail(QV2X_EINVAL, "qv2x_pfn_scatter_i8: lanes per pillar 0 (the library's choice) | 16 | 64");
+    if (lanes == 16 && max_points > PFN_SLOTS) return fail(QV2X_EINVAL, "qv2x_pfn_scatter_i8: the 16-lane form takes max_points <= %d", PFN_SLOTS);
     if (M == 0) return QV2X_OK;
     if (!voxel_features || !voxel_coords || !voxel_num_points || !params || !canvas)
         return fail(QV2X_EINVAL, "qv2x_pfn_scatter_i8: null pointer");
     if (M < 0 || max_points <= 0 || N <= 0 || ny <= 0 || nx <= 0) return fail(QV2X_EINVAL, "qv2x_pfn_scatter_i8: bad sizes");
     if (((uintptr_t)voxel_features & 15) || ((uintptr_t)voxel_coords & 15)) return fail(QV2X_EALIGN, "qv2x_pfn_scatter_i8: inputs must be 16-byte aligned");
-    int form = 16;
+    int form = lanes ? lanes : max_points > PFN_SLOTS ? 64 : 16;
 #ifdef QV2X_DEV_KNOBS
-    static const int form_env = getenv("QV2X_PFN_FORM") ? atoi(getenv("QV2X_PFN_FORM")) : 16;
-    form = form_env;
+    static const int form_env = getenv("QV2X_PFN_FORM") ? atoi(getenv("QV2X_PFN_FORM")) : 0;
+    if (!lanes && form_env == 64) form = 64;
 #endif
     if (form == 64)
         pfn_scatter_kernel<<<(M + 4 * PFN_PB - 1) / (4 * PFN_PB), 256, 0, (hipStream_t)stream>>>((const float4*)voxel_features, (const int4*)voxel_coords,
diff --git a/quantv2x_amd/encode_two_stage.py b/quantv2x_amd/encode_two_stage.py
--- a/quantv2x_amd/encode_two_stage.py
+++ b/quantv2x_amd/encode_two_stage.py
@@ -91,6 +91,7 @@
 
 
 CANDIDATE_ENTRY = {128: "qv2x_codebook_encode_candidates_i8", 256: "qv2x_codebook_encode_candidates_seg_i8"}
+CANDIDATE_ENTRY_CLEARED = {128: "qv2x_codebook_encode_candidates_cleared_i8", 256: "qv2x_codebook_encode_candidates_seg_cleared_i8"}
 
 
 def candidate_tables(state: Dict[str, np.ndarray], levels: int, in_delta: float, in_zx: int, segs: int = 1) -> Dict[str, np.ndarray]:
diff --git a/quantv2x_amd/engine.py b/quantv2x_amd/engine.py
--- a/quantv2x_amd/engine.py
+++ b/quantv2x_amd/engine.py
@@ -640,16 +640,23 @@
             L.check(self.lib.qv2x_fill_i8(L.ptr(b["canvas"]), b["canvas"].numel(), int(self.pfn.z2) - 128, L.current_stream()), "qv2x_fill_i8")
             b["canvas_clean"] = True
 
-    def clear_pillars(self, inputs: dict, n_agents: int):
+    def clear_pillars(self, inputs: dict, n_agents: int, reset_encode_counters: bool = False) -> bool:
         if self.encoder_kind == "second":
-            return
+            return False
         b = self._workspace(n_agents)
         co = inputs["voxel_coords"].to(torch.int32).contiguous()
+        if reset_encode_counters and self.encode_mode == "two_stage" and self.encode_form == "auto" and self._two_stage is not None:
+            cnt = b["enc_counters"]
+            L.check(self.lib.qv2x_pfn_unscatter_reset_i8(L.ptr(co), co.shape[0], int(self.pfn.z2) - 128, L.ptr(b["canvas"]), n_agents, self.ny, self.nx,
+                                                         L.ptr(cnt), cnt.numel(), L.current_stream()), "qv2x_pfn_unscatter_reset_i8")
+            b["canvas_clean"] = True
+            return True
         L.check(self.lib.qv2x_pfn_unscatter_i8(L.ptr(co), co.shape[0], int(self.pfn.z2) - 128, L.ptr(b["canvas"]), n_agents, self.ny, self.nx,
                                                L.current_stream()), "qv2x_pfn_unscatter_i8")
         b["canvas_clean"] = True
-
-    def encode_codes(self, n_agents: int, out: Optional[torch.Tensor] = None):
+        return False
+
+    def encode_codes(self, n_agents: int, out: Optional[torch.Tensor] = None, counters_clear: bool = False):
         b = self._workspace(n_agents)
         codes = b["codes"] if out is None else out
         if codes.dtype != torch.uint8 or not codes.is_contiguous() or codes.numel() != self.levels * n_agents * self.fh * self.fw:
@@ -673,7 +680,7 @@
                                                                 L.current_stream()), "qv2x_codebook_encode_collapsed_f32")
             return codes
         if two_stage:
-            return self._encode_two_stage(d, b, codes)
+            return self._encode_two_stage(d, b, codes, counters_clear)
         if self.encode_mode not in ("exact", "two_stage"):
             raise ValueError(f"encode_mode {self.encode_mode!r}: 'exact' (every cell through the reference's op order), 'two_stage' (the same "
                              "indices: exact integer candidates, the chain only where the bound cannot decide) or 'collapsed' (opt-in, approximate)")
@@ -711,13 +718,13 @@
         except Exception as e:
             self.encode_mode, self.two_stage_refused = "exact", str(e) or type(e).__name__
 
-    def candidate_entry(self) -> str:
-        from .encode_two_stage import CANDIDATE_ENTRY, pack_factor
-        return CANDIDATE_ENTRY[pack_factor(self.segs, self.kc)]
-
-    def _encode_two_stage(self, d, b, codes):
+    def candidate_entry(self, counters_clear: bool = False) -> str:
+        from .encode_two_stage import CANDIDATE_ENTRY, CANDIDATE_ENTRY_CLEARED, pack_factor
+        return (CANDIDATE_ENTRY_CLEARED if counters_clear else CANDIDATE_ENTRY)[pack_factor(self.segs, self.kc)]
+
+    def _encode_two_stage(self, d, b, codes, counters_clear: bool = False):
         gp, bias, tab, tau, _ = self._two_stage
-        name = self.candidate_entry()
+        name = self.candidate_entry(counters_clear)
         L.check(getattr(self.lib, name)(C.byref(d), L.ptr(b["s1"]), L.ptr(gp), L.ptr(bias), L.ptr(tab), tau, L.ptr(codes),
                                         L.ptr(b["enc_list"]), L.ptr(b["enc_counters"]), L.current_stream()), name)
         L.check(self.lib.qv2x_codebook_encode_listed_f32(C.byref(d), L.ptr(b["s1"]), self.level_ptrs, L.ptr(b["enc_list"]), L.ptr(b["enc_counters"]),
@@ -740,11 +747,11 @@
         self.pillars_to_canvas(inputs, frames, resident=True)
         try:
             self.run_plan(frames)
-            self.clear_pillars(inputs, frames)
+            cleared = self.clear_pillars(inputs, frames, reset_encode_counters=True)
         except BaseException:
             self._restore_canvas(frames)
             raise
-        return self.encode_codes(frames, out=codes_out)
+        return self.encode_codes(frames, out=codes_out, counters_clear=cleared)
 
     def pairwise_from_poses(self, gathered: torch.Tensor, world: int, agent_stride: int, pose_offset: int, max_cav: int, out: torch.Tensor):
         L.check(self.lib.qv2x_pairwise_from_poses_f64(L.ptr(gathered), world, agent_stride, pose_offset, max_cav, L.ptr(out),
@@ -828,7 +835,7 @@
             self.run_plan(n_agents, taps=taps)
             if taps is not None:
                 taps["canvas"], taps["cat"] = canvas.clone(), b["cat"]
-            self.clear_pillars(inputs, n_agents)
+            cleared = self.clear_pillars(inputs, n_agents, reset_encode_counters=self.has_codebook)
         except BaseException:
             self._restore_canvas(n_agents)
             raise
@@ -837,7 +844,7 @@
         if taps is not None and self.compress:
             for c, out in zip(self.comp, b["comp"]):
                 taps[c.name] = out
-        return self.encode_codes(n_agents) if self.has_codebook else (b["comp"][-1] if self.compress else b["s1"])
+        return self.encode_codes(n_agents, counters_clear=cleared) if self.has_codebook else (b["comp"][-1] if self.compress else b["s1"])
 
     def decode_rows(self, codes, n_rows_total):
         out = torch.empty((n_rows_total, 256), dtype=torch.float32, device=self.dev)
diff --git a/quantv2x_amd/lib.py b/quantv2x_amd/lib.py
--- a/quantv2x_amd/lib.py
+++ b/quantv2x_amd/lib.py
@@ -24,6 +24,8 @@
     "qv2x_fuse_att_band_f32", "qv2x_heads_band", "qv2x_fuse_heads_band", "qv2x_assemble_bands",
     "qv2x_voxelize_batch_workspace_bytes", "qv2x_voxelize_batch_f32", "qv2x_postprocess_batch_workspace_bytes", "qv2x_postprocess_batch_f32",
     "qv2x_eval_workspace_bytes", "qv2x_eval_tp_fp_f32", "qv2x_gt_boxes_f32",
+    "qv2x_pfn_scatter_form_i8", "qv2x_pfn_fetch_slot", "qv2x_pfn_unscatter_reset_i8",
+    "qv2x_codebook_encode_candidates_cleared_i8", "qv2x_codebook_encode_candidates_seg_cleared_i8",
 ]
 WIRES = {"f32": 0, "u8": 1}
 COMM_ID_BYTES = 128
@@ -146,6 +148,9 @@
     lib.qv2x_fill_i8.argtypes = [vp, C.c_int64, C.c_int, vp]
     lib.qv2x_pfn_scatter_i8.argtypes = [vp, vp, vp, C.c_int, C.c_int, C.POINTER(PfnParams), vp, C.c_int, C.c_int, C.c_int, vp]
     lib.qv2x_pfn_unscatter_i8.argtypes = [vp, C.c_int, C.c_int, vp, C.c_int, C.c_int, C.c_int, vp]
+    lib.qv2x_pfn_scatter_form_i8.argtypes = [vp, vp, vp, C.c_int, C.c_int, C.POINTER(PfnParams), vp, C.c_int, C.c_int, C.c_int, C.c_int, vp]
+    lib.qv2x_pfn_fetch_slot.argtypes = [C.c_int, C.c_int, C.c_int, C.c_int]
+    lib.qv2x_pfn_unscatter_reset_i8.argtypes = [vp, C.c_int, C.c_int, vp, C.c_int, C.c_int, C.c_int, vp, C.c_int, vp]
     lib.qv2x_conv3x3_i8.argtypes = [C.POINTER(ConvDesc), vp, vp, vp, vp, vp, vp, vp, vp]
     lib.qv2x_conv3x3_i8_wide.argtypes = [C.POINTER(ConvDesc), vp, vp, vp, vp, vp, vp, vp, vp]
     lib.qv2x_conv3x3_i8_chain64.argtypes = [C.POINTER(ChainDesc), vp, vp, vp, vp, vp, vp, vp, vp]
@@ -173,6 +178,8 @@
     lib.qv2x_codebook_encode_collapsed_f32.argtypes = [C.POINTER(EncodeDesc), vp, vp, vp, vp, vp, vp]
     lib.qv2x_codebook_encode_candidates_i8.argtypes = [C.POINTER(EncodeDesc), vp, vp, vp, vp, C.POINTER(C.c_float), vp, vp, vp, vp]
     lib.qv2x_codebook_encode_candidates_seg_i8.argtypes = [C.POINTER(EncodeDesc), vp, vp, vp, vp, C.POINTER(C.c_float), vp, vp, vp, vp]
+    lib.qv2x_codebook_encode_candidates_cleared_i8.argtypes = lib.qv2x_codebook_encode_candidates_i8.argtypes
+    lib.qv2x_codebook_encode_candidates_seg_cleared_i8.argtypes = lib.qv2x_codebook_encode_candidates_seg_i8.argtypes
     lib.qv2x_codebook_encode_listed_f32.argtypes = [C.POINTER(EncodeDesc), vp, C.POINTER(vp), vp, vp, vp, vp]
     lib.qv2x_mean_vfe_f32.argtypes = [vp, vp, vp, C.c_int, C.c_int, vp, vp]
     lib.qv2x_sp_index_scatter.argtypes = [vp, vp, C.c_int, C.c_int, C.c_int, C.c_int, C.c_int, vp, C.c_int, vp]
```

New measurement: 6969, median of 6. 1.01x the previous value.
